# tohtsky/myFM

Hardware: AMD Instinct MI355X
Metric: Gibbs iterations/sec (rank=32) (higher is better)
Workload: dtype f64

## Files before the change

### myfm_amd/csrc/mfm_res.hpp

```cpp
#pragma once
#include <algorithm>
#include <cstdlib>
#include <cstring>
#include <atomic>
#include <string>
#include <thread>
#include <vector>

#include "mfm_common.hpp"
#include "mfm_mf_kernels.hpp"

namespace mfm {

#ifndef MFM_RES_CH
#define MFM_RES_CH 4
#endif
constexpr int RES_MAX_PEERS = 8;

struct ResArgs {
  double2 *eq;
  const double *e_in;
  double *e_slots;
  const int32_t *perm;
  const uint32_t *uidw;
  const uint32_t *headw;
  const int32_t *run_item;
  const int32_t *first_run;
  const int32_t *wg_run_ptr;
  const int32_t *wg_nruns;
  const int32_t *wg_user_ptr;
  const int2 *user_desc;
  const int32_t *wg_item_ptr;
  const int32_t *ent_ptr;
  const int2 *entries;
  const int32_t *scols;
  const int2 *item_desc;
  double *partials;
  double *dv;
  double *V;
  int64_t D;
  int f_begin, f_end;
  int linear;
  int n_sw;
  double *w;
  const double *zw;
  const double *lam_w, *mu_w;
  double e_shift;
  const double *z;
  const double *lam, *mu;
  const int32_t *group;
  int n_groups;
  double alpha;
  const double *scal;
  int n_items, umax;
  unsigned long long *bar;
  int n_wg;
  int *error;
  unsigned long long *prof;
  int xworld, xrank;
  unsigned long long xepoch0;
  double *xsum[RES_MAX_PEERS];
  unsigned long long *xflag[RES_MAX_PEERS];
  unsigned long long *xarrive;
  int xmodel;
  double *xw[RES_MAX_PEERS], *xV[RES_MAX_PEERS];
  int ngx;
  int no_store;
  int xch_break;
};

__device__ __forceinline__ void res_store2(double *p, double a, double b) {
  __hip_atomic_store(p, a, __ATOMIC_RELAXED, __HIP_MEMORY_SCOPE_AGENT);
  __hip_atomic_store(p + 1, b, __ATOMIC_RELAXED, __HIP_MEMORY_SCOPE_AGENT);
}

enum { RES_BAR_START = 0, RES_BAR_TOP = 16, RES_BAR_XCNT = 32, RES_BAR_GEN = 160, RES_BAR_CENSUS = 288, RES_BAR_WORDS = 416 };
struct ResBar {
  int xcc;
  unsigned long long n_x, nx;
};

__device__ __forceinline__ bool res_spin(const ResArgs &a, const unsigned long long *w, unsigned long long target, bool &dead) {
  unsigned spins = 0;
  while (__hip_atomic_load(w, __ATOMIC_RELAXED, __HIP_MEMORY_SCOPE_AGENT) < target) {
#ifndef MFM_RES_NO_SLEEP
    __builtin_amdgcn_s_sleep(1);
#endif
    if ((++spins & 1023u) == 0u) {
      if (spins > (1u << 22) || __hip_atomic_load(a.error, __ATOMIC_RELAXED, __HIP_MEMORY_SCOPE_AGENT) != 0) {
        __hip_atomic_store(a.error, 1, __ATOMIC_RELAXED, __HIP_MEMORY_SCOPE_AGENT);
        dead = true;
        return false;
      }
    }
  }
  return true;
}

__device__ __forceinline__ bool res_spin_sys(const ResArgs &a, const unsigned long long *w, unsigned long long target, bool &dead) {
  unsigned spins = 0;
  while (__hip_atomic_load(w, __ATOMIC_RELAXED, __HIP_MEMORY_SCOPE_SYSTEM) < target) {
    __builtin_amdgcn_s_sleep(2);
    if ((++spins & 1023u) == 0u) {
      const int seen = __hip_atomic_load(a.error, __ATOMIC_RELAXED, __HIP_MEMORY_SCOPE_AGENT);
      if (spins > (1u << 23) || seen != 0) {
        if (seen == 0) __hip_atomic_store(a.error, 2, __ATOMIC_RELAXED, __HIP_MEMORY_SCOPE_AGENT);
        dead = true;
        return false;
      }
    }
  }
  return true;
}

__device__ __forceinline__ void res_bar_init(const ResArgs &a, ResBar &rb, bool &dead) {
  unsigned x;
  asm volatile("s_getreg_b32 %0, hwreg(HW_REG_XCC_ID, 0, 4)" : "=s"(x));
  rb.xcc = (int)(x & 7u);
  __hip_atomic_fetch_add(a.bar + RES_BAR_CENSUS + 16 * rb.xcc, 1ull, __ATOMIC_RELAXED, __HIP_MEMORY_SCOPE_AGENT);
  asm volatile("s_waitcnt vmcnt(0)" ::: "memory");
  __hip_atomic_fetch_add(a.bar + RES_BAR_START, 1ull, __ATOMIC_RELAXED, __HIP_MEMORY_SCOPE_AGENT);
  rb.n_x = 1;
  rb.nx = 1;
  if (!res_spin(a, a.bar + RES_BAR_START, (unsigned long long)a.n_wg, dead)) return;
  rb.nx = 0;
  for (int i = 0; i < 8; i++) {
    const unsigned long long c = __hip_atomic_load(a.bar + RES_BAR_CENSUS + 16 * i, __ATOMIC_RELAXED, __HIP_MEMORY_SCOPE_AGENT);
    rb.nx += c > 0 ? 1 : 0;
    if (i == rb.xcc) rb.n_x = c;
  }
}

__device__ __forceinline__ void res_grid_barrier(const ResArgs &a, const ResBar &rb, unsigned long long k, int tid, bool &dead) {
  asm volatile("s_waitcnt vmcnt(0)" ::: "memory");
  __syncthreads();
  if (tid == 0 && !dead) {
    const unsigned long long old =
        __hip_atomic_fetch_add(a.bar + RES_BAR_XCNT + 16 * rb.xcc, 1ull, __ATOMIC_RELAXED, __HIP_MEMORY_SCOPE_AGENT);
    if (old + 1 == k * rb.n_x) {
      __builtin_amdgcn_fence(__ATOMIC_RELEASE, "agent");
      asm volatile("s_waitcnt vmcnt(0)" ::: "memory");
      __hip_atomic_fetch_add(a.bar + RES_BAR_TOP, 1ull, __ATOMIC_RELAXED, __HIP_MEMORY_SCOPE_AGENT);
      if (res_spin(a, a.bar + RES_BAR_TOP, k * rb.nx, dead))
        __hip_atomic_store(a.bar + RES_BAR_GEN + 16 * rb.xcc, k, __ATOMIC_RELAXED, __HIP_MEMORY_SCOPE_AGENT);
    } else {
      res_spin(a, a.bar + RES_BAR_GEN + 16 * rb.xcc, k, dead);
    }
    __builtin_amdgcn_fence(__ATOMIC_ACQUIRE, "agent");
  }
  __syncthreads();
}

typedef double res_d16_t __attribute__((ext_vector_type(16)));
typedef unsigned res_u4_t __attribute__((ext_vector_type(4)));

template <int NT, int NGV, int NGL, bool XCH = false, bool OVF = false>
__global__ __launch_bounds__(NT) void k_mf_resident(ResArgs a) {
  extern __shared__ __attribute__((aligned(16))) char res_smem[];
  constexpr int NW = NT / WAVE, NG = NGV + NGL, R = 16 * NG, RL = 16 * NGL;
  constexpr int B = 4;
  const int g = (int)blockIdx.x, tid = threadIdx.x, lane = tid & 63;
  const int wv = __builtin_amdgcn_readfirstlane(tid >> 6);
  const int U = a.umax;
  const double alpha_k = a.scal ? a.scal[0] : a.alpha, e_shift_k = a.scal ? a.scal[2] : a.e_shift;
  const int ngx = OVF ? a.ngx : 0, NGt = NG + ngx, Rt = 16 * NGt;
  double *elds = (double *)res_smem;
  double *acc1 = elds + (size_t)RL * NT;
  double *acc2 = acc1 + NW * U;
  d2_t *utab = (d2_t *)(acc2 + NW * U);
  d2_t *wcarry = utab + U;
  int *wflag = (int *)(wcarry + NW);
  const int32_t *perm_g = a.perm + (int64_t)g * Rt * NT;
  const d2_t *dv2 = (const d2_t *)a.dv;
  const int u0 = a.wg_user_ptr[g], nu = a.wg_user_ptr[g + 1] - u0;
  const int rb0 = a.wg_run_ptr[g];
  const int pad_item = a.n_items;
  bool dead = false;
  unsigned long long nbar = 0;
  ResBar rbar;
  rbar.xcc = 0;
  rbar.n_x = rbar.nx = 1;
#define RES_STAMP0(k) \
  if (a.prof && tid == 0) a.prof[(int64_t)g * a.n_sw * 64 + 56 + (k)] = __builtin_amdgcn_s_memrealtime()
  RES_STAMP0(0);
  if (tid == 0) res_bar_init(a, rbar, dead);
  RES_STAMP0(1);
  const int wv_hi = wv >> 2;
#define RES_PRIO(j)                  \
  if ((((j) & 1) ^ wv_hi) != 0)      \
    __builtin_amdgcn_s_setprio(1);   \
  else                               \
    __builtin_amdgcn_s_setprio(0)
  const int trash_run = a.wg_run_ptr[g] + a.wg_nruns[g];
#define RES_STAMP(k)                                                                                      \
  if (a.prof && tid == 0) a.prof[((int64_t)g * a.n_sw + (f - f_first)) * 64 + (k)] = __builtin_amdgcn_s_memrealtime()

  for (int i = tid; i < 2 * NW * U; i += NT) acc1[i] = 0.0;
  for (int i = tid; i < U; i += NT) utab[i] = d2_t{0.0, 0.0};

  res_u4_t uw[NG];
  unsigned ux[NG];
  unsigned hbv[NG], nbv[NG];
#pragma unroll
  for (int j = 0; j < NG; j++) {
#pragma unroll
    for (int w = 0; w < 4; w++) uw[j][w] = a.uidw[((int64_t)g * (5 * NGt) + 5 * j + w) * NT + tid];
    ux[j] = a.uidw[((int64_t)g * (5 * NGt) + 5 * j + 4) * NT + tid];
    hbv[j] = a.headw[((int64_t)g * NGt + j) * NT + tid];
    nbv[j] = hbv[j] | (j == 0 ? 1u : 0u);
  }
  const unsigned nbx0 = OVF && ngx > 0 ? a.headw[((int64_t)g * NGt + NG) * NT + tid] : 0u;
  double *eog = OVF ? a.e_slots + ((int64_t)g * Rt + 16 * NG) * NT + tid : nullptr;
  const uint32_t *uidw_x = a.uidw + ((int64_t)g * (5 * NGt) + 5 * NG) * NT + tid;
  const uint32_t *headw_x = a.headw + ((int64_t)g * NGt + NG) * NT + tid;
  const int run0 = a.first_run[g * NT + tid];
  const bool head0 = (hbv[0] & 1u) != 0u;
#define RES_NIB(j, q) ((((nbv[j]) | ((j) + 1 < NG ? nbv[(j) + 1 < NG ? (j) + 1 : (j)] << 16 : nbx0 << 16)) >> (4 * (q))) & 15u)
#define RES_UIDS(j, bb, uid)                                                     \
  {                                                                              \
    const unsigned lo_ = uw[j][bb];                                              \
    uid[0] = (int)(lo_ & 0x3ffu);                                                \
    uid[1] = (int)((lo_ >> 10) & 0x3ffu);                                        \
    uid[2] = (int)((lo_ >> 20) & 0x3ffu);                                        \
    uid[3] = (int)((lo_ >> 30) | (((ux[j] >> (8 * (bb))) & 0xffu) << 2));        \
  }

#define RES_UIDSX(bb, uid)                                                       \
  {                                                                              \
    const unsigned lo_ = uwx[bb];                                                \
    uid[0] = (int)(lo_ & 0x3ffu);                                                \
    uid[1] = (int)((lo_ >> 10) & 0x3ffu);                                        \
    uid[2] = (int)((lo_ >> 20) & 0x3ffu);                                        \
    uid[3] = (int)((lo_ >> 30) | (((uxx >> (8 * (bb))) & 0xffu) << 2));          \
  }

  res_d16_t ev[NGV > 0 ? NGV : 1];
#pragma unroll
  for (int j = 0; j < NG; j++) {
#pragma unroll 1
    for (int bb = 0; bb < 4; bb++) {
      int row[B];
#pragma unroll
      for (int k = 0; k < B; k++) row[k] = a.e_in ? 0 : perm_g[(16 * j + 4 * bb + k) * NT + tid];
#pragma unroll
      for (int k = 0; k < B; k++) {
        const double x = (a.e_in ? a.e_in[((int64_t)g * Rt + 16 * j + 4 * bb + k) * NT + tid] : a.eq[row[k] < 0 ? 0 : row[k]].x) + e_shift_k;
        if (j < NGV)
          ev[j < NGV ? j : 0][4 * bb + k] = x;
        else
          elds[(16 * (j - NGV) + 4 * bb + k) * NT + tid] = x;
      }
    }
  }
  if (OVF) {
    for (int jx = 0; jx < ngx; jx++) {
#pragma unroll 4
      for (int i = 0; i < 16; i++) {
        const int64_t sl = 16 * (NG + jx) + i;
        const int row = a.e_in ? 0 : perm_g[sl * NT + tid];
        const double x = (a.e_in ? a.e_in[((int64_t)g * Rt + sl) * NT + tid] : a.eq[row < 0 ? 0 : row].x) + e_shift_k;
        eog[(16 * jx + i) * NT] = x;
      }
    }
  }
  __syncthreads();

  RES_STAMP0(2);
  const int f_first = a.f_begin - a.linear;
  for (int f = f_first; f < a.f_end; f++) {
    const bool lin = f < a.f_begin;
    double *Vf = lin ? a.w : a.V + (int64_t)f * a.D;
    const double *zf = lin ? a.zw : a.z + (int64_t)(f - a.f_begin) * a.D;
    const double *lamf = lin ? a.lam_w : a.lam + (int64_t)f * a.n_groups;
    const double *muf = lin ? a.mu_w : a.mu + (int64_t)f * a.n_groups;
    int uj = 0;
    double uold = 0.0, uz = 0.0, ulam = 0.0, umu = 0.0;
    if (tid < nu) {
      const int2 d = a.user_desc[u0 + tid];
      uj = d.x;
      uold = Vf[uj];
      uz = zf[uj];
      ulam = lamf[d.y];
      umu = muf[d.y];
    }
    RES_STAMP(0);
    {
      int rc = run0 - 1;
      int itA[B];
      d2_t ddA[B];
      {
        int it0[B];
        const unsigned n0 = RES_NIB(0, 0), n1 = RES_NIB(0, 1);
#pragma unroll
        for (int k = 0; k < B; k++) {
          rc += (int)((n0 >> k) & 1u);
          it0[k] = a.run_item[(n0 >> k) & 1u ? rc : rb0];
        }
#pragma unroll
        for (int k = 0; k < B; k++) {
          rc += (int)((n1 >> k) & 1u);
          itA[k] = a.run_item[(n1 >> k) & 1u ? rc : rb0];
        }
#pragma unroll
        for (int k = 0; k < B; k++) ddA[k] = dv2[(n0 >> k) & 1u ? it0[k] : pad_item];
      }
      d2_t ddc = d2_t{0.0, 0.0};
      int itB[B];
      d2_t ddB[B];
#define RES_STEP_A(j, bb, iti, ito, ddi, ddo)                                                                              \
  {                                                                                                                        \
    const unsigned n4 = RES_NIB(j, bb), n4a = RES_NIB(j, (bb) + 1), n4b = RES_NIB(j, (bb) + 2);                            \
    _Pragma("unroll") for (int k = 0; k < B; k++) {                                                                        \
      rc += (int)((n4b >> k) & 1u);                                                                                        \
      ito[k] = a.run_item[(n4b >> k) & 1u ? rc : rb0];                                                                     \
    }                                                                                                                      \
    _Pragma("unroll") for (int k = 0; k < B; k++) ddo[k] = dv2[(n4a >> k) & 1u ? iti[k] : pad_item];                       \
    int uid[B];                                                                                                            \
    RES_UIDS(j, bb, uid);                                                                                                  \
    double up[B], ex[B];                                                                                                   \
    _Pragma("unroll") for (int k = 0; k < B; k++) {                                                                        \
      up[k] = utab[uid[k]][0];                                                                                             \
      ex[k] = j < NGV ? ev[j < NGV ? j : 0][4 * (bb) + k] : elds[(16 * (j - NGV) + 4 * (bb) + k) * NT + tid];              \
    }                                                                                                                      \
    _Pragma("unroll") for (int k = 0; k < B; k++) {                                                                        \
      const bool need = ((n4 >> k) & 1u) != 0u;                                                                            \
      ddc[0] = need ? ddi[k][0] : ddc[0];                                                                                  \
      ddc[1] = need ? ddi[k][1] : ddc[1];                                                                                  \
      const double er = ex[k] + up[k] * ddc[0];                                                                            \
      if (j < NGV)                                                                                                         \
        ev[j < NGV ? j : 0][4 * (bb) + k] = er;                                                                            \
      else                                                                                                                 \
        elds[(16 * (j - NGV) + 4 * (bb) + k) * NT + tid] = er;                                                             \
      const double c = ddc[1];                                                                                             \
      __hip_atomic_fetch_add(&acc1[wv * U + uid[k]], (-er) * c, __ATOMIC_RELAXED, __HIP_MEMORY_SCOPE_WORKGROUP);           \
      __hip_atomic_fetch_add(&acc2[wv * U + uid[k]], c * c, __ATOMIC_RELAXED, __HIP_MEMORY_SCOPE_WORKGROUP);               \
    }                                                                                                                      \
  }
#define RES_STEP_AX(bb, iti, ito, ddi, ddo)                                                                                 \
  {                                                                                                                        \
    const unsigned n4 = ((nbw >> (4 * (bb))) & 15u), n4a = ((nbw >> (4 * ((bb) + 1))) & 15u), n4b = ((nbw >> (4 * ((bb) + 2))) & 15u);                            \
    _Pragma("unroll") for (int k = 0; k < B; k++) {                                                                        \
      rc += (int)((n4b >> k) & 1u);                                                                                        \
      ito[k] = a.run_item[(n4b >> k) & 1u ? rc : rb0];                                                                     \
    }                                                                                                                      \
    _Pragma("unroll") for (int k = 0; k < B; k++) ddo[k] = dv2[(n4a >> k) & 1u ? iti[k] : pad_item];                       \
    int uid[B];                                                                                                            \
    RES_UIDSX(bb, uid);                                                                                                      \
    double up[B], ex[B];                                                                                                   \
    _Pragma("unroll") for (int k = 0; k < B; k++) {                                                                        \
      up[k] = utab[uid[k]][0];                                                                                             \
      ex[k] = eo[4 * (bb) + k];              \
    }                                                                                                                      \
    _Pragma("unroll") for (int k = 0; k < B; k++) {                                                                        \
      const bool need = ((n4 >> k) & 1u) != 0u;                                                                            \
      ddc[0] = need ? ddi[k][0] : ddc[0];                                                                                  \
      ddc[1] = need ? ddi[k][1] : ddc[1];                                                                                  \
      const double er = ex[k] + up[k] * ddc[0];                                                                            \
      eo[4 * (bb) + k] = er;                                                             \
      const double c = ddc[1];                                                                                             \
      __hip_atomic_fetch_add(&acc1[wv * U + uid[k]], (-er) * c, __ATOMIC_RELAXED, __HIP_MEMORY_SCOPE_WORKGROUP);           \
      __hip_atomic_fetch_add(&acc2[wv * U + uid[k]], c * c, __ATOMIC_RELAXED, __HIP_MEMORY_SCOPE_WORKGROUP);               \
    }                                                                                                                      \
  }
#pragma unroll
      for (int j = 0; j < NG; j++) {
        RES_PRIO(j);
#pragma unroll 1
        for (int bp = 0; bp < 2; bp++) {
          RES_STEP_A(j, 2 * bp, itA, itB, ddA, ddB);
          RES_STEP_A(j, 2 * bp + 1, itB, itA, ddB, ddA);
        }
      }
      if (OVF) {
        unsigned hb_c = nbx0;
        for (int jx = 0; jx < ngx; jx++) {
          res_u4_t uwx;
#pragma unroll
          for (int w = 0; w < 4; w++) uwx[w] = uidw_x[(5 * jx + w) * NT];
          const unsigned uxx = uidw_x[(5 * jx + 4) * NT];
          const unsigned hb_n = jx + 1 < ngx ? headw_x[(jx + 1) * NT] : 0u;
          const unsigned nbw = hb_c | (hb_n << 16);
          res_d16_t eo;
#pragma unroll
          for (int i = 0; i < 16; i++) eo[i] = eog[(16 * jx + i) * NT];
#pragma unroll 1
          for (int bp = 0; bp < 2; bp++) {
            RES_STEP_AX(2 * bp, itA, itB, ddA, ddB);
            RES_STEP_AX(2 * bp + 1, itB, itA, ddB, ddA);
          }
#pragma unroll
          for (int i = 0; i < 16; i++) eog[(16 * jx + i) * NT] = eo[i];
          hb_c = hb_n;
        }
      }
#undef RES_STEP_A
#undef RES_STEP_AX
    }
    __syncthreads();
    RES_STAMP(1);
    if (tid < nu) {
      double S1 = 0.0, S2 = 0.0;
#pragma unroll
      for (int w = 0; w < NW; w++) {
        S1 += acc1[w * U + tid];
        S2 += acc2[w * U + tid];
        acc1[w * U + tid] = 0.0;
        acc2[w * U + tid] = 0.0;
      }
      const double fresh = PMainV::draw(S1, S2, uold, alpha_k, ulam, umu, uz);
      Vf[uj] = fresh;
      if (XCH && a.xmodel) {
        for (int r = 0; r < a.xworld; r++)
          if (r != a.xrank)
            __hip_atomic_store((lin ? a.xw[r] : a.xV[r] + (int64_t)f * a.D) + uj, fresh, __ATOMIC_RELAXED, __HIP_MEMORY_SCOPE_SYSTEM);
      }
      utab[tid] = d2_t{lin ? 1.0 : fresh, fresh - uold};
    }
    __syncthreads();
    RES_STAMP(2);
    {
      bool have_head = false;
      double f1 = 0.0, f2 = 0.0, s1 = 0.0, s2 = 0.0;
      d2_t *part2 = (d2_t *)a.partials;
      {
        int rc = run0 - 1, rcC = run0 - 1;
        int itA[B];
        double ccA[B];
        {
          int it0[B];
          const unsigned n0 = RES_NIB(0, 0), n1 = RES_NIB(0, 1);
#pragma unroll
          for (int k = 0; k < B; k++) {
            rc += (int)((n0 >> k) & 1u);
            it0[k] = a.run_item[(n0 >> k) & 1u ? rc : rb0];
          }
#pragma unroll
          for (int k = 0; k < B; k++) {
            rc += (int)((n1 >> k) & 1u);
            itA[k] = a.run_item[(n1 >> k) & 1u ? rc : rb0];
          }
#pragma unroll
          for (int k = 0; k < B; k++) ccA[k] = a.dv[2 * (int64_t)((n0 >> k) & 1u ? it0[k] : pad_item) + 1];
        }
        double ccc = 0.0;
        int itB[B];
        double ccB[B];
#ifdef MFM_RES_UCST
#define RES_PARTIAL_STORE() part2[head && have_head ? rcC - 1 : trash_run] = d2_t{s1, s2}
#else
#define RES_PARTIAL_STORE() \
  if (head && have_head) part2[rcC - 1] = d2_t{s1, s2}
#endif
#define RES_STEP_B(j, bb, iti, ito, cci, cco)                                                                              \
  {                                                                                                                        \
    const unsigned n4 = RES_NIB(j, bb), n4a = RES_NIB(j, (bb) + 1), n4b = RES_NIB(j, (bb) + 2);                            \
    const unsigned h4 = (hbv[j] >> (4 * (bb))) & 15u;                                                                      \
    _Pragma("unroll") for (int k = 0; k < B; k++) {                                                                        \
      rc += (int)((n4b >> k) & 1u);                                                                                        \
      ito[k] = a.run_item[(n4b >> k) & 1u ? rc : rb0];                                                                     \
    }                                                                                                                      \
    _Pragma("unroll") for (int k = 0; k < B; k++) cco[k] = a.dv[2 * (int64_t)((n4a >> k) & 1u ? iti[k] : pad_item) + 1];   \
    int uid[B];                                                                                                            \
    RES_UIDS(j, bb, uid);                                                                                                  \
    d2_t ut[B];                                                                                                            \
    double ex[B];                                                                                                          \
    _Pragma("unroll") for (int k = 0; k < B; k++) {                                                                        \
      ut[k] = utab[uid[k]];                                                                                                \
      ex[k] = j < NGV ? ev[j < NGV ? j : 0][4 * (bb) + k] : elds[(16 * (j - NGV) + 4 * (bb) + k) * NT + tid];              \
    }                                                                                                                      \
    _Pragma("unroll") for (int k = 0; k < B; k++) {                                                                        \
      const bool need = ((n4 >> k) & 1u) != 0u;                                                                            \
      const bool head = ((h4 >> k) & 1u) != 0u;                                                                            \
      ccc = need ? cci[k] : ccc;                                                                                           \
      rcC += need ? 1 : 0;                                                                       \
                              \
      RES_PARTIAL_STORE();                                                                                                 \
      f1 = head && !have_head ? s1 : f1;                                                                                   \
      f2 = head && !have_head ? s2 : f2;                                                                                   \
      have_head = have_head || head;                                                                                       \
      const double er = ex[k] + ccc * ut[k][1];                                                                            \
      if (j < NGV)                                                                                                         \
        ev[j < NGV ? j : 0][4 * (bb) + k] = er;                                                                            \
      else                                                                                                                 \
        elds[(16 * (j - NGV) + 4 * (bb) + k) * NT + tid] = er;                                                             \
      s1 = (head ? 0.0 : s1) + (-er) * ut[k][0];                                                                           \
      s2 = (head ? 0.0 : s2) + ut[k][0] * ut[k][0];                                                                        \
    }                                                                                                                      \
  }
#define RES_STEP_BX(bb, iti, ito, cci, cco)                                                                                 \
  {                                                                                                                        \
    const unsigned n4 = ((nbw >> (4 * (bb))) & 15u), n4a = ((nbw >> (4 * ((bb) + 1))) & 15u), n4b = ((nbw >> (4 * ((bb) + 2))) & 15u);                            \
    const unsigned h4 = (hb_c >> (4 * (bb))) & 15u;                                                                       \
    _Pragma("unroll") for (int k = 0; k < B; k++) {                                                                        \
      rc += (int)((n4b >> k) & 1u);                                                                                        \
      ito[k] = a.run_item[(n4b >> k) & 1u ? rc : rb0];                                                                     \
    }                                                                                                                      \
    _Pragma("unroll") for (int k = 0; k < B; k++) cco[k] = a.dv[2 * (int64_t)((n4a >> k) & 1u ? iti[k] : pad_item) + 1];   \
    int uid[B];                                                                                                            \
    RES_UIDSX(bb, uid);                                                                                                      \
    d2_t ut[B];                                                                                                            \
    double ex[B];                                                                                                          \
    _Pragma("unroll") for (int k = 0; k < B; k++) {                                                                        \
      ut[k] = utab[uid[k]];                                                                                                \
      ex[k] = eo[4 * (bb) + k];              \
    }                                                                                                                      \
    _Pragma("unroll") for (int k = 0; k < B; k++) {                                                                        \
      const bool need = ((n4 >> k) & 1u) != 0u;                                                                            \
      const bool head = ((h4 >> k) & 1u) != 0u;                                                                            \
      ccc = need ? cci[k] : ccc;                                                                                           \
      rcC += need ? 1 : 0;                                                                       \
                              \
      RES_PARTIAL_STORE();                                                                                                 \
      f1 = head && !have_head ? s1 : f1;                                                                                   \
      f2 = head && !have_head ? s2 : f2;                                                                                   \
      have_head = have_head || head;                                                                                       \
      const double er = ex[k] + ccc * ut[k][1];                                                                            \
      eo[4 * (bb) + k] = er;                                                             \
      s1 = (head ? 0.0 : s1) + (-er) * ut[k][0];                                                                           \
      s2 = (head ? 0.0 : s2) + ut[k][0] * ut[k][0];                                                                        \
    }                                                                                                                      \
  }
#pragma unroll
        for (int j = 0; j < NG; j++) {
          RES_PRIO(j);
#pragma unroll 1
          for (int bp = 0; bp < 2; bp++) {
              RES_STEP_B(j, 2 * bp, itA, itB, ccA, ccB);
            if (a.prof && lane == 0 && (wv == 4 || wv == 7))
              a.prof[((int64_t)g * a.n_sw + (f - f_first)) * 64 + 16 + (wv == 4 ? 0 : 20) + 4 * j + 2 * bp] =
                  __builtin_amdgcn_s_memrealtime();
            RES_STEP_B(j, 2 * bp + 1, itB, itA, ccB, ccA);
            if (a.prof && lane == 0 && (wv == 4 || wv == 7))
              a.prof[((int64_t)g * a.n_sw + (f - f_first)) * 64 + 16 + (wv == 4 ? 0 : 20) + 4 * j + 2 * bp + 1] =
                  __builtin_amdgcn_s_memrealtime();
          }
        }
        if (OVF) {
          unsigned hb_c = nbx0;
          for (int jx = 0; jx < ngx; jx++) {
            res_u4_t uwx;
#pragma unroll
            for (int w = 0; w < 4; w++) uwx[w] = uidw_x[(5 * jx + w) * NT];
            const unsigned uxx = uidw_x[(5 * jx + 4) * NT];
            const unsigned hb_n = jx + 1 < ngx ? headw_x[(jx + 1) * NT] : 0u;
            const unsigned nbw = hb_c | (hb_n << 16);
            res_d16_t eo;
#pragma unroll
            for (int i = 0; i < 16; i++) eo[i] = eog[(16 * jx + i) * NT];
#pragma unroll 1
            for (int bp = 0; bp < 2; bp++) {
              RES_STEP_BX(2 * bp, itA, itB, ccA, ccB);
              RES_STEP_BX(2 * bp + 1, itB, itA, ccB, ccA);
            }
#pragma unroll
            for (int i = 0; i < 16; i++) eog[(16 * jx + i) * NT] = eo[i];
            hb_c = hb_n;
          }
        }
#undef RES_STEP_B
#undef RES_STEP_BX
#undef RES_PARTIAL_STORE
      }
      if (a.prof && lane == 0)
        a.prof[((int64_t)g * a.n_sw + (f - f_first)) * 64 + 8 + wv] = __builtin_amdgcn_s_memrealtime();
      double v1 = s1, v2 = s2;
      int fl = have_head ? 1 : 0;
      wave_segscan2(v1, v2, fl);
      if (lane == 63) {
        wcarry[wv] = d2_t{v1, v2};
        wflag[wv] = fl;
      }
      double x1 = dpp_f64<0x138, 0xf>(v1), x2 = dpp_f64<0x138, 0xf>(v2);
      int xf = dpp_i32<0x138, 0xf>(fl, 0);
      if (lane == 0) {
        x1 = 0.0;
        x2 = 0.0;
        xf = 0;
      }
      lds_barrier();
      if (have_head && tid > 0) {
        if (!xf) {
          double c1 = 0.0, c2 = 0.0;
          for (int w = 0; w < wv; w++) {
            const d2_t cw = wcarry[w];
            const bool fw = wflag[w] != 0;
            c1 = (fw ? 0.0 : c1) + cw[0];
            c2 = (fw ? 0.0 : c2) + cw[1];
          }
          x1 = c1 + x1;
          x2 = c2 + x2;
        }
        const int closing = head0 ? run0 - 1 : run0;
        part2[closing] = d2_t{x1 + f1, x2 + f2};
      }
    }
    RES_STAMP(3);
    constexpr int CH = MFM_RES_CH;
    const int c0 = a.ent_ptr[g] >> 6, c1 = a.ent_ptr[g + 1] >> 6;
    const int per = (c1 - c0 + NW - 1) / NW;
    const int wb = c0 + wv * per, we = wb + per < c1 ? wb + per : c1;
    const int i0 = a.wg_item_ptr[g], ni = a.wg_item_ptr[g + 1] - i0;
    const bool more = f + 1 < a.f_end;
    int ij = 0;
    double iold = 0.0, iz = 0.0, ivn = 0.0, ilam = 0.0, imu = 0.0;
    if (tid < ni) {
      const int2 d = a.item_desc[i0 + tid];
      ij = d.x;
      iold = Vf[ij];
      iz = zf[ij];
      ivn = more ? a.V[(int64_t)(f + 1) * a.D + ij] : 0.0;
      ilam = lamf[d.y];
      imu = muf[d.y];
    }
    int2 en[CH];
#pragma unroll
    for (int k = 0; k < CH; k++) en[k] = make_int2(0, 0);
    if (wb < we) {
#pragma unroll
      for (int k = 0; k < CH; k++) en[k] = a.entries[(int64_t)(wb + k < we ? wb + k : wb) * WAVE + lane];
    }
    res_grid_barrier(a, rbar, ++nbar, tid, dead);
    RES_STAMP(4);
    {
      const d2_t *part2 = (const d2_t *)a.partials;
      for (int cb = wb; cb < we; cb += CH) {
        d2_t sv[CH];
#pragma unroll
        for (int k = 0; k < CH; k++) sv[k] = part2[en[k].x];
        int il[CH];
#pragma unroll
        for (int k = 0; k < CH; k++) il[k] = en[k].y;
        if (cb + CH < we) {
#pragma unroll
          for (int k = 0; k < CH; k++) en[k] = a.entries[(int64_t)(cb + CH + k < we ? cb + CH + k : cb + CH) * WAVE + lane];
        }
#pragma unroll
        for (int k = 0; k < CH; k++) {
          if (cb + k >= we) break;
          __hip_atomic_fetch_add(&acc1[wv * U + il[k]], sv[k][0], __ATOMIC_RELAXED, __HIP_MEMORY_SCOPE_WORKGROUP);
          __hip_atomic_fetch_add(&acc2[wv * U + il[k]], sv[k][1], __ATOMIC_RELAXED, __HIP_MEMORY_SCOPE_WORKGROUP);
        }
      }
      __syncthreads();
      double S1 = 0.0, S2 = 0.0;
      if (tid < ni) {
#pragma unroll
        for (int w = 0; w < NW; w++) {
          S1 += acc1[w * U + tid];
          S2 += acc2[w * U + tid];
          acc1[w * U + tid] = 0.0;
          acc2[w * U + tid] = 0.0;
        }
      }
      if (XCH) {
        const unsigned long long E = a.xepoch0 + (unsigned long long)(f - f_first) + 1ull;
        const int64_t stride = 2 * ((int64_t)a.n_items + 1), par = (int64_t)(E & 1ull);
        if (tid < ni) {
          const int64_t off = ((int64_t)a.xrank * 2 + par) * stride + 2 * (int64_t)(i0 + tid);
          for (int r = 0; r < a.xworld; r++) {
            __hip_atomic_store(a.xsum[r] + off, S1, __ATOMIC_RELAXED, __HIP_MEMORY_SCOPE_SYSTEM);
            __hip_atomic_store(a.xsum[r] + off + 1, S2, __ATOMIC_RELAXED, __HIP_MEMORY_SCOPE_SYSTEM);
          }
        }
        asm volatile("s_waitcnt vmcnt(0)" ::: "memory");
        __syncthreads();
        if (tid == 0 && !dead) {
          const unsigned long long old = __hip_atomic_fetch_add(a.xarrive, 1ull, __ATOMIC_RELAXED, __HIP_MEMORY_SCOPE_AGENT);
          if (old + 1 == (unsigned long long)a.n_wg * E) {
            for (int r = 0; r < a.xworld && !a.xch_break; r++)
              __hip_atomic_store(a.xflag[r] + 16 * a.xrank, E, __ATOMIC_RELEASE, __HIP_MEMORY_SCOPE_SYSTEM);
          }
          for (int r = 0; r < a.xworld && !dead; r++) res_spin_sys(a, a.xflag[a.xrank] + 16 * r, E, dead);
        }
        __syncthreads();
        if (tid < ni) {
          S1 = S2 = 0.0;
          for (int r = 0; r < a.xworld; r++) {
            const int64_t off = ((int64_t)r * 2 + par) * stride + 2 * (int64_t)(i0 + tid);
            S1 += __hip_atomic_load(a.xsum[a.xrank] + off, __ATOMIC_RELAXED, __HIP_MEMORY_SCOPE_SYSTEM);
            S2 += __hip_atomic_load(a.xsum[a.xrank] + off + 1, __ATOMIC_RELAXED, __HIP_MEMORY_SCOPE_SYSTEM);
          }
        }
      }
      if (tid < ni) {
        const double fresh = PMainV::draw(S1, S2, iold, alpha_k, ilam, imu, iz);
        Vf[ij] = fresh;
        res_store2(a.dv + 2 * (int64_t)(i0 + tid), fresh - iold, ivn);
      }
    }
    RES_STAMP(5);
    res_grid_barrier(a, rbar, ++nbar, tid, dead);
    RES_STAMP(6);
  }
#undef RES_STAMP
  RES_STAMP0(3);
  if (!a.no_store) {
    int run_last = run0;
#pragma unroll
    for (int j = 0; j < NG; j++) {
#pragma unroll 1
      for (int bb = 0; bb < 4; bb++) {
        const unsigned h4 = (hbv[j] >> (4 * bb)) & 15u;
        int row[B], it[B];
#pragma unroll
        for (int k = 0; k < B; k++) {
          if (16 * j + 4 * bb + k > 0) run_last += (int)((h4 >> k) & 1u);
          it[k] = a.run_item[run_last];
          row[k] = perm_g[(16 * j + 4 * bb + k) * NT + tid];
        }
        int uid[B];
        RES_UIDS(j, bb, uid);
#pragma unroll
        for (int k = 0; k < B; k++) {
          const double dl = a.dv[2 * (int64_t)it[k]];
          const double ex = j < NGV ? ev[j < NGV ? j : 0][4 * bb + k] : elds[(16 * (j - NGV) + 4 * bb + k) * NT + tid];
          const double ef = ex + utab[uid[k]][0] * dl;
          if (a.e_slots)
            a.e_slots[((int64_t)g * Rt + 16 * j + 4 * bb + k) * NT + tid] = ef;
          else if (row[k] >= 0)
            a.eq[row[k]].x = ef;
        }
      }
    }
    if (OVF) {
      for (int jx = 0; jx < ngx; jx++) {
        res_u4_t uwx;
#pragma unroll
        for (int w = 0; w < 4; w++) uwx[w] = uidw_x[(5 * jx + w) * NT];
        const unsigned uxx = uidw_x[(5 * jx + 4) * NT];
        const unsigned hbx = headw_x[jx * NT];
#pragma unroll 1
        for (int bb = 0; bb < 4; bb++) {
          const unsigned h4 = (hbx >> (4 * bb)) & 15u;
          int it[B], uid[B];
#pragma unroll
          for (int k = 0; k < B; k++) {
            run_last += (int)((h4 >> k) & 1u);
            it[k] = a.run_item[run_last];
          }
          RES_UIDSX(bb, uid);
#pragma unroll
          for (int k = 0; k < B; k++) {
            const double dl = a.dv[2 * (int64_t)it[k]];
            double *ep = eog + (16 * jx + 4 * bb + k) * NT;
            *ep = *ep + utab[uid[k]][0] * dl;
          }
        }
      }
    }
  }
#undef RES_PRIO
#undef RES_NIB
#undef RES_UIDS
#undef RES_UIDSX
  asm volatile("s_waitcnt vmcnt(0)" ::: "memory");
  RES_STAMP0(4);
#undef RES_STAMP0
}

__global__ void k_res_init_dv(const double *__restrict__ theta, const int32_t *__restrict__ scols, int n_items,
                              double *__restrict__ dv, unsigned long long *__restrict__ bar) {
  const int i = blockIdx.x * blockDim.x + threadIdx.x;
  if (blockIdx.x == 0)
    for (int k = threadIdx.x; k < RES_BAR_WORDS; k += blockDim.x) bar[k] = 0ull;
  if (i < n_items) {
    dv[2 * i] = 0.0;
    dv[2 * i + 1] = theta ? theta[scols[i]] : 1.0;
  } else if (i == n_items) {
    dv[2 * i] = 0.0;
    dv[2 * i + 1] = 0.0;
  }
}

__global__ void k_res_unpermute(const double *__restrict__ e_slots, const int32_t *__restrict__ perm, int64_t n_slots,
                                double2 *__restrict__ eq) {
  const int64_t i = (int64_t)blockIdx.x * blockDim.x + threadIdx.x;
  if (i >= n_slots) return;
  const int32_t row = perm[i];
  if (row >= 0) eq[row].x = e_slots[i];
}

struct ResScoreArgs {
  const uint32_t *uidw, *headw;
  const int32_t *first_run, *run_feat, *wg_user_ptr, *wg_fill;
  const int2 *user_desc;
  int umax, KS;
  const double *Vt, *w;
  double w0;
  const double *w0p;
  const double *y_slots;
  double *e_slots;
  double2 *sums;
  unsigned long long *prof;
};

template <int NT, int NG, int KPT>
__global__ __launch_bounds__(NT) void k_res_score(ResScoreArgs a) {
  extern __shared__ __attribute__((aligned(16))) char res_smem[];
  constexpr int R = 16 * NG, NW = NT / WAVE;
  constexpr int US = 2 * KPT + 2;
  const int g = blockIdx.x, tid = threadIdx.x, lane = tid & 63, wv = tid >> 6;
  const int KP = a.KS >> 1;
  const double w0_k = a.w0p ? *a.w0p : a.w0;
  double *uV = (double *)res_smem;
  double *uW = uV + (size_t)a.umax * US;
  double2 *wsum = (double2 *)(uW + ((a.umax + 1) & ~1));
  if (a.prof && tid == 0) a.prof[4 * g] = __builtin_amdgcn_s_memrealtime();
  int *ucol = (int *)(wsum + NW);
  const int u0 = a.wg_user_ptr[g], nu = a.wg_user_ptr[g + 1] - u0;
  for (int ul = tid; ul < a.umax; ul += NT) {
    const int ju = ul < nu ? a.user_desc[u0 + ul].x : -1;
    ucol[ul] = ju;
    uW[ul] = ju >= 0 ? a.w[ju] : 0.0;
  }
  __syncthreads();
#pragma unroll 4
  for (int i = tid; i < a.umax * KPT; i += NT) {
    const int ul = i / KPT, pr = i - ul * KPT;
    const int ju = ucol[ul];
    double2 v = make_double2(0.0, 0.0);
    if (ju >= 0 && pr < KP) v = ((const double2 *)(a.Vt + (int64_t)ju * a.KS))[pr];
    ((double2 *)(uV + (size_t)ul * US))[pr] = v;
  }
  res_u4_t uw[NG];
  unsigned ux[NG], hbv[NG];
#pragma unroll
  for (int j = 0; j < NG; j++) {
#pragma unroll
    for (int w = 0; w < 4; w++) uw[j][w] = a.uidw[((int64_t)g * (5 * NG) + 5 * j + w) * NT + tid];
    ux[j] = a.uidw[((int64_t)g * (5 * NG) + 5 * j + 4) * NT + tid];
    hbv[j] = a.headw[((int64_t)g * NG + j) * NT + tid];
  }
  int run = a.first_run[g * NT + tid];
  const int64_t fill = a.wg_fill[g];
  __syncthreads();
  if (a.prof && tid == 0) a.prof[4 * g + 1] = __builtin_amdgcn_s_memrealtime();
  double2 vi[KPT];
  double wi = 0.0, s1 = 0.0, s2 = 0.0;
#pragma unroll
  for (int p = 0; p < KPT; p++) vi[p] = make_double2(0.0, 0.0);
  int jc[4], jn[4];
  double yn[4];
#pragma unroll
  for (int k = 0; k < 4; k++) yn[k] = a.y_slots[((int64_t)g * R + k) * NT + tid];
  {
    const unsigned h0 = hbv[0] & 15u;
    int r = run;
#pragma unroll
    for (int k = 0; k < 4; k++) {
      if (k > 0) r += (int)((h0 >> k) & 1u);
      jc[k] = a.run_feat[r];
    }
    run = r;
  }
#pragma unroll
  for (int j = 0; j < NG; j++) {
    const unsigned hb2 = hbv[j] | (j + 1 < NG ? hbv[j + 1 < NG ? j + 1 : j] << 16 : 0u);
#pragma unroll 1
    for (int bb = 0; bb < 4; bb++) {
      {
        const unsigned hn = (hb2 >> (4 * (bb + 1))) & 15u;
        int r = run;
#pragma unroll
        for (int k = 0; k < 4; k++) {
          r += (int)((hn >> k) & 1u);
          jn[k] = a.run_feat[r];
        }
        run = r;
      }
      const unsigned lo_ = uw[j][bb];
      int uid[4];
      uid[0] = (int)(lo_ & 0x3ffu);
      uid[1] = (int)((lo_ >> 10) & 0x3ffu);
      uid[2] = (int)((lo_ >> 20) & 0x3ffu);
      uid[3] = (int)((lo_ >> 30) | (((ux[j] >> (8 * bb)) & 0xffu) << 2));
      const unsigned h4 = (hbv[j] >> (4 * bb)) & 15u;
      double yv[4], eb[4];
#pragma unroll
      for (int k = 0; k < 4; k++) yv[k] = yn[k];
      {
        const int nb = 16 * j + 4 * bb + 4 < R ? 16 * j + 4 * bb + 4 : 0;
#pragma unroll
        for (int k = 0; k < 4; k++) yn[k] = a.y_slots[((int64_t)g * R + nb + k) * NT + tid];
      }
#pragma unroll
      for (int k = 0; k < 4; k++) {
        const int slot = 16 * j + 4 * bb + k;
        const bool head = slot == 0 || ((h4 >> k) & 1u);
        if (head) {
          const int ji = jc[k];
          wi = 0.0;
          if (ji >= 0) {
            const double2 *src = (const double2 *)(a.Vt + (int64_t)ji * a.KS);
#pragma unroll
            for (int p = 0; p < KPT; p++) vi[p] = p < KP ? src[p] : make_double2(0.0, 0.0);
            wi = a.w[ji];
          } else {
#pragma unroll
            for (int p = 0; p < KPT; p++) vi[p] = make_double2(0.0, 0.0);
          }
        }
        const double2 *vu = (const double2 *)(uV + (size_t)uid[k] * US);
        double d0 = 0.0, d1 = 0.0;
#pragma unroll
        for (int p = 0; p < KPT; p += 2) {
          const double2 x0 = vu[p], x1 = vu[p + 1];
          d0 += x0.x * vi[p].x + x0.y * vi[p].y;
          d1 += x1.x * vi[p + 1].x + x1.y * vi[p + 1].y;
        }
        const double pred = w0_k + (uW[uid[k]] + wi) + (d0 + d1);
        const bool real = (int64_t)tid * R + slot < fill;
        const double e = real ? pred - yv[k] : 0.0;
        eb[k] = e;
        s1 += e;
        s2 += e * e;
      }
#pragma unroll
      for (int k = 0; k < 4; k++) a.e_slots[((int64_t)g * R + 16 * j + 4 * bb + k) * NT + tid] = eb[k];
#pragma unroll
      for (int k = 0; k < 4; k++) jc[k] = jn[k];
    }
  }
  if (a.prof && lane == 0) a.prof[4 * g + 2] = __builtin_amdgcn_s_memrealtime();
  wave_allreduce_sum2(s1, s2);
  if (lane == 0) wsum[wv] = make_double2(s1, s2);
  __syncthreads();
  if (a.prof && tid == 0) a.prof[4 * g + 3] = __builtin_amdgcn_s_memrealtime();
  if (tid == 0) {
    double t1 = 0.0, t2 = 0.0;
    for (int w = 0; w < NW; w++) {
      t1 += wsum[w].x;
      t2 += wsum[w].y;
    }
    a.sums[g] = make_double2(t1, t2);
  }
}

__global__ void k_res_permute_y(const double *__restrict__ y, const int32_t *__restrict__ perm, int64_t n_slots,
                                double *__restrict__ y_slots) {
  const int64_t i = (int64_t)blockIdx.x * blockDim.x + threadIdx.x;
  if (i >= n_slots) return;
  const int32_t row = perm[i];
  y_slots[i] = row >= 0 ? y[row] : 0.0;
}

template <class F>
static inline void res_parallel_for(int n, F f) {
  const int hw = (int)std::thread::hardware_concurrency();
  const int T = std::max(1, std::min({n, 16, hw > 0 ? hw : 1}));
  if (T == 1) {
    for (int i = 0; i < n; i++) f(i);
    return;
  }
  std::atomic<int> next(0);
  auto work = [&]() {
    for (;;) {
      const int i = next.fetch_add(1);
      if (i >= n) return;
      f(i);
    }
  };
  std::vector<std::thread> pool;
  for (int t = 1; t < T; t++) pool.emplace_back(work);
  work();
  for (auto &t : pool) t.join();
}

struct ResPlan {
  bool ready = false;
  int G = 0, NT = 512, RV = 0, RL = 0, umax = 0, item_bits = 0, n_items = 0;
  int RX = 0;
  int R() const { return RV + RL + RX; }
  bool allow_overflow = true;
  int64_t n_rows = 0, n_runs = 0;
  size_t lds_bytes = 0;
  DevBuf<int32_t> perm, first_run, wg_run_ptr, wg_nruns, wg_user_ptr, wg_item_ptr, ent_ptr, scols;
  DevBuf<int2> entries;
  DevBuf<uint32_t> uidw, headw;
  DevBuf<int32_t> run_item;
  DevBuf<int2> user_desc, item_desc;
  DevBuf<double> partials, dv, e_slots;
  DevBuf<unsigned long long> bar;
  DevBuf<int32_t> run_feat, wg_fill;
  DevBuf<double> y_slots;
  DevBuf<double2> sums;
  int maxu_rows = 0;
  int xworld = 1, xrank = 0;
  bool peers_set = false;
  DevBuf<double> xsum;
  DevBuf<unsigned long long> xflag, xarrive;
  double *peer_sum[RES_MAX_PEERS] = {nullptr, nullptr, nullptr, nullptr, nullptr, nullptr, nullptr, nullptr};
  unsigned long long *peer_flag[RES_MAX_PEERS] = {nullptr, nullptr, nullptr, nullptr, nullptr, nullptr, nullptr, nullptr};
  unsigned long long xepoch = 0;
  bool peers_model = false;
  double *peer_w[RES_MAX_PEERS] = {nullptr, nullptr, nullptr, nullptr, nullptr, nullptr, nullptr, nullptr};
  double *peer_V[RES_MAX_PEERS] = {nullptr, nullptr, nullptr, nullptr, nullptr, nullptr, nullptr, nullptr};
  std::vector<void *> peer_mapped;
  size_t xsum_bytes(int world) const { return (size_t)world * 2 * 2 * ((size_t)n_items + 1) * sizeof(double); }
  void alloc_exchange(int world, int rank, hipStream_t s) {
    xworld = world;
    xrank = rank;
    peers_set = false;
    peers_model = false;
    xepoch = 0;
    auto alloc_shared = [&](auto &buf, size_t count) {
      buf.release();
      void *p = nullptr;
      const size_t bytes = count * sizeof(*buf.p);
      if (hipExtMallocWithFlags(&p, bytes, hipDeviceMallocUncached) != hipSuccess) {
        (void)hipGetLastError();
        throw Error(MFM_ERR_DEVICE, "no uncached device memory for the ranks' exchange buffers (hipExtMallocWithFlags(hipDeviceMallocUncached))");
      }
      buf.p = (decltype(buf.p))p;
      buf.n = count;
      buf.owned = true;
      MFM_HIP_CHECK(hipMemsetAsync(p, 0, bytes, s));
    };
    alloc_shared(xsum, xsum_bytes(world) / sizeof(double));
    alloc_shared(xflag, (size_t)16 * RES_MAX_PEERS);
    xarrive.alloc_zero(16, s);
  }
  std::string why;
  std::vector<int32_t> h_nruns;
  std::vector<std::string> h_diag;

  static int bits_for(int64_t n) {
    int b = 1;
    while (((int64_t)1 << b) < n) b++;
    return b;
  }
  struct Variant {
    int rv, rl;
  };
  static const Variant *variants(int &n) {
    static const Variant v[] = {{16, 0}, {32, 0}, {64, 16}};
    n = 3;
    return v;
  }

  bool choose_layout(int64_t N, const std::vector<int64_t> &ustart, int64_t max_user, int n_cu, std::vector<int64_t> &ucut) {
    const int64_t n_users = (int64_t)ustart.size() - 1;
    int nv = 0;
    const Variant *vs = variants(nv);
    bool found = false;
    for (int vi = 0; vi < nv && !found; vi++) {
      const int64_t cap = (int64_t)NT * (vs[vi].rv + vs[vi].rl) - 1;
      if (max_user > cap) continue;
      const int64_t slack = std::min<int64_t>(cap / 8, max_user);
      int64_t Gw = (N + (cap - slack) - 1) / (cap - slack);
      if (Gw > n_cu && N <= (int64_t)n_cu * cap) Gw = n_cu;
      if (Gw > n_cu) continue;
      if (env_flag("MFM_RES_WGS")) Gw = std::min<int64_t>(n_cu, std::max<int64_t>(Gw, env_i64("MFM_RES_WGS", 0)));
      Gw = std::min<int64_t>(Gw, n_users);
      ucut.assign(1, 0);
      bool ok = true;
      for (int64_t g = 1; g <= Gw && ok; g++) {
        const int64_t lo_u = ucut.back();
        int64_t hi_u;
        if (g == Gw) {
          hi_u = n_users;
        } else {
          const int64_t want = (N * g) / Gw;
          hi_u = std::upper_bound(ustart.begin(), ustart.end(), want) - ustart.begin() - 1;
          if (hi_u + 1 <= n_users && ustart[hi_u + 1] - want < want - ustart[hi_u]) hi_u++;
          hi_u = std::max(hi_u, lo_u + 1);
          hi_u = std::min<int64_t>(hi_u, n_users - (Gw - g));
          while (hi_u > lo_u + 1 && ustart[hi_u] - ustart[lo_u] > cap) hi_u--;
        }
        if (hi_u <= lo_u || ustart[hi_u] - ustart[lo_u] > cap) ok = false;
        ucut.push_back(hi_u);
      }
      if (!ok) continue;
      G = (int)Gw;
      RV = vs[vi].rv;
      RL = vs[vi].rl;
      found = true;
    }
    RX = 0;
    if (!found && allow_overflow) {
      const Variant big = vs[nv - 1];
      for (int rx = 16; rx <= 80 && !found; rx += 16) {
        const int64_t cap = (int64_t)NT * (big.rv + big.rl + rx) - 1;
        if (max_user > cap || N > (int64_t)n_cu * cap) continue;
        int64_t Gw = std::min<int64_t>(n_cu, n_users);
        ucut.assign(1, 0);
        bool ok = true;
        for (int64_t g = 1; g <= Gw && ok; g++) {
          const int64_t lo_u = ucut.back();
          int64_t hi_u;
          if (g == Gw) {
            hi_u = n_users;
          } else {
            const int64_t want = (N * g) / Gw;
            hi_u = std::upper_bound(ustart.begin(), ustart.end(), want) - ustart.begin() - 1;
            if (hi_u + 1 <= n_users && ustart[hi_u + 1] - want < want - ustart[hi_u]) hi_u++;
            hi_u = std::max(hi_u, lo_u + 1);
            hi_u = std::min<int64_t>(hi_u, n_users - (Gw - g));
            while (hi_u > lo_u + 1 && ustart[hi_u] - ustart[lo_u] > cap) hi_u--;
          }
          if (hi_u <= lo_u || ustart[hi_u] - ustart[lo_u] > cap) ok = false;
          ucut.push_back(hi_u);
        }
        if (!ok) continue;
        G = (int)Gw;
        RV = big.rv;
        RL = big.rl;
        RX = rx;
        found = true;
      }
    }
    if (!found) return fail("no variant fits (rows per CU, or a first-level column longer than a workgroup's capacity)");
    return true;
  }
  bool choose_item_slices(const std::vector<int32_t> &slot_ptr, int64_t counter, std::vector<int32_t> &iptr) {
    iptr.assign((size_t)G + 1, 0);
    bool ok = false;
    for (double scale = 1.0; scale < 3.0 && !ok; scale *= 1.1) {
      const double target = scale * ((double)counter + 16.0 * n_items) / G;
      double acc = 0.0;
      int gq = 0, cnt = 0;
      for (int c = 0; c < n_items; c++) {
        acc += (double)(slot_ptr[c + 1] - slot_ptr[c]) + 16.0;
        cnt++;
        if ((acc >= target || cnt == NT) && gq + 1 < G) {
          iptr[++gq] = c + 1;
          acc = 0.0;
          cnt = 0;
        }
      }
      ok = cnt <= NT;
      for (gq++; gq <= G; gq++) iptr[gq] = n_items;
    }
    if (!ok) return fail("more second-level columns than the workgroups can draw");
    return true;
  }
  static std::vector<int32_t> run_bases(const std::vector<int32_t> &nruns) {
    const int G = (int)nruns.size();
    std::vector<int32_t> run_base((size_t)G + 1, 0);
    for (int g = 0; g < G; g++) run_base[g + 1] = run_base[g] + nruns[g] + 1;
    return run_base;
  }

  bool build(const HostCsr &csc, const std::vector<int32_t> &level, const std::vector<int32_t> *group_of, int n_cu,
             const std::vector<char> *draw_empty = nullptr) {
    ready = false;
    const int64_t N = csc.cols, D0 = csc.rows;
    n_rows = N;
    if (N < 1 || n_cu < 1 || (int64_t)level.size() != D0) return fail("shape");
    std::vector<int32_t> users, items, empties;
    for (int64_t j = 0; j < D0; j++) {
      if (level[j] == 0) {
        if (csc.ptr[j + 1] > csc.ptr[j])
          users.push_back((int32_t)j);
        else if (!draw_empty || (*draw_empty)[(size_t)j])
          empties.push_back((int32_t)j);
      } else if (level[j] == 1) {
        items.push_back((int32_t)j);
      } else {
        return fail("more than two levels");
      }
    }
    n_items = (int)items.size();
    if (users.empty() || items.empty()) return fail("empty level");
    std::sort(users.begin(), users.end(), [&](int32_t x, int32_t y) { return csc.idx[csc.ptr[x]] < csc.idx[csc.ptr[y]]; });
    std::vector<int64_t> ustart(users.size() + 1);
    int64_t next_row = 0, max_user = 0;
    for (size_t u = 0; u < users.size(); u++) {
      const int32_t j = users[u];
      const int64_t b = csc.ptr[j], len = csc.ptr[j + 1] - b;
      if (csc.idx[b] != next_row || csc.idx[b + len - 1] != next_row + len - 1) return fail("first level not contiguous");
      ustart[u] = next_row;
      next_row += len;
      max_user = std::max(max_user, len);
    }
    ustart[users.size()] = next_row;
    if (next_row != N) return fail("first level does not cover the rows");
    std::vector<int32_t> item_of_row((size_t)N, -1);
    {
      int64_t cnt = 0;
      for (int c = 0; c < n_items; c++) cnt += csc.ptr[items[c] + 1] - csc.ptr[items[c]];
      if (cnt != N) return fail("second level does not cover the rows");
      const int chunks = std::max(1, std::min(n_items, 64));
      res_parallel_for(chunks, [&](int k) {
        for (int c = (int)((int64_t)n_items * k / chunks); c < (int)((int64_t)n_items * (k + 1) / chunks); c++)
          for (int64_t p = csc.ptr[items[c]]; p < csc.ptr[items[c] + 1]; p++) item_of_row[csc.idx[p]] = c;
      });
      std::atomic<bool> bad(false);
      res_parallel_for(chunks, [&](int k) {
        for (int64_t r = N * k / chunks; r < N * (k + 1) / chunks; r++)
          if (item_of_row[r] < 0) bad = true;
      });
      if (bad) return fail("second level touches a row twice");
    }
    std::vector<int64_t> ucut;
    if (!choose_layout(N, ustart, max_user, n_cu, ucut)) return false;
    const int R = RV + RL + RX;
    const int64_t cap_slots = (int64_t)NT * R;
    std::vector<std::vector<int32_t>> wg_users((size_t)G);
    for (int g = 0; g < G; g++)
      for (int64_t u = ucut[g]; u < ucut[g + 1]; u++) wg_users[g].push_back(users[u]);
    for (size_t k = 0; k < empties.size(); k++) wg_users[k % G].push_back(empties[k]);
    int maxu = 0;
    for (int g = 0; g < G; g++) maxu = std::max(maxu, (int)wg_users[g].size());
    if (maxu > NT) return fail("more first-level columns in a workgroup than threads");
    item_bits = bits_for((int64_t)n_items + 1);
    const int UW = 5 * (R / 16), HW = R / 16;
    std::vector<uint16_t> h_uid((size_t)G * cap_slots, 0xffffu);
    std::vector<uint32_t> h_headw((size_t)G * HW * NT, 0);
    std::vector<int32_t> h_perm((size_t)G * cap_slots, -1), h_first((size_t)G * NT, 0);
    std::vector<std::vector<int32_t>> wg_run_item((size_t)G);
    std::vector<int64_t> fill((size_t)G, 0);
    std::vector<int32_t> nruns((size_t)G, 0);
    res_parallel_for(G, [&](int g) {
      const int64_t row0 = ustart[ucut[g]], row1 = ustart[ucut[g + 1]];
      const int64_t n = row1 - row0;
      std::vector<int32_t> cnt((size_t)n_items + 1, 0), uloc((size_t)n);
      for (int64_t u = ucut[g]; u < ucut[g + 1]; u++)
        for (int64_t r = ustart[u]; r < ustart[u + 1]; r++) uloc[(size_t)(r - row0)] = (int32_t)(u - ucut[g]);
      for (int64_t r = row0; r < row1; r++) cnt[(size_t)item_of_row[r] + 1]++;
      std::vector<int32_t> &runs = wg_run_item[g];
      for (int c = 0; c < n_items; c++) {
        if (cnt[c + 1]) {
          const int64_t sidx = cnt[c];
          const int th = (int)(sidx / R), rh = (int)(sidx % R);
          h_headw[((size_t)g * HW + rh / 16) * NT + th] |= 1u << (rh % 16);
          runs.push_back(c);
        }
        cnt[c + 1] += cnt[c];
      }
      {
        size_t ri = 0;
        std::vector<int32_t> run_start(runs.size());
        for (size_t k = 0; k < runs.size(); k++) run_start[k] = cnt[runs[k]];
        for (int t = 0; t < NT; t++) {
          const int64_t s0 = (int64_t)t * R;
          if (s0 >= n) break;
          while (ri + 1 < runs.size() && run_start[ri + 1] <= s0) ri++;
          h_first[(size_t)g * NT + t] = (int32_t)ri;
        }
      }
      for (int64_t r = row0; r < row1; r++) {
        const int64_t sidx = cnt[(size_t)item_of_row[r]]++;
        const int t = (int)(sidx / R), rr = (int)(sidx % R);
        h_perm[(size_t)g * cap_slots + (size_t)rr * NT + t] = (int32_t)r;
        h_uid[(size_t)g * cap_slots + (size_t)sidx] = (uint16_t)uloc[(size_t)(r - row0)];
      }
      fill[g] = n;
      nruns[g] = (int32_t)runs.size();
    });
    std::vector<int32_t> h_slot_ptr((size_t)n_items + 1, 0);
    int64_t counter = 0;
    for (int g = 0; g < G; g++) {
      counter += nruns[g];
      for (int32_t c : wg_run_item[g]) h_slot_ptr[(size_t)c + 1]++;
    }
    for (int c = 0; c < n_items; c++) h_slot_ptr[(size_t)c + 1] += h_slot_ptr[c];
    h_slot_ptr[n_items] = (int32_t)counter;
    n_runs = counter;
    if (counter >= ((int64_t)1 << 31) - 2) return fail("too many runs");
    std::vector<int32_t> run_base = run_bases(nruns);
    const int32_t zero_run = run_base[G];
    std::vector<int32_t> h_run_item((size_t)zero_run + 1, n_items);
    for (int g = 0; g < G; g++) {
      std::copy(wg_run_item[g].begin(), wg_run_item[g].end(), h_run_item.begin() + run_base[g]);
      if (fill[g] < cap_slots) {
        const int th = (int)(fill[g] / R), rh = (int)(fill[g] % R);
        h_headw[((size_t)g * HW + rh / 16) * NT + th] |= 1u << (rh % 16);
      }
      h_headw[((size_t)g * HW) * NT] |= 1u;
      for (int t = 0; t < NT; t++) {
        const int64_t s0 = (int64_t)t * R;
        int32_t &fr = h_first[(size_t)g * NT + t];
        fr = (s0 >= fill[g] ? nruns[g] : fr) + run_base[g];
      }
    }
    std::vector<int32_t> h_uptr((size_t)G + 1, 0);
    std::vector<int2> h_udesc;
    for (int g = 0; g < G; g++) {
      for (int32_t j : wg_users[g]) h_udesc.push_back(make_int2(j, group_of && (size_t)j < group_of->size() ? (*group_of)[j] : 0));
      h_uptr[g + 1] = (int32_t)h_udesc.size();
    }
    std::vector<int32_t> h_iptr;
    if (!choose_item_slices(h_slot_ptr, counter, h_iptr)) return false;
    int imax = 0;
    for (int g = 0; g < G; g++) imax = std::max(imax, h_iptr[g + 1] - h_iptr[g]);
    umax = std::max(maxu, imax) + 1;
    if (umax > 1024) return fail("internal: user field");
    std::vector<uint32_t> h_uidw((size_t)G * UW * NT, 0);
    res_parallel_for(G, [&](int g) {
      for (int64_t sl = 0; sl < cap_slots; sl++) {
        const uint16_t u16 = h_uid[(size_t)g * cap_slots + (size_t)sl];
        const uint32_t u = u16 == 0xffffu ? (uint32_t)(umax - 1) : u16;
        const int t = (int)(sl / R), r = (int)(sl % R);
        const int w0 = 5 * (r / 16), bb = (r % 16) / 4, k = r % 4;
        if (k < 3) {
          h_uidw[((size_t)g * UW + w0 + bb) * NT + t] |= u << (10 * k);
        } else {
          h_uidw[((size_t)g * UW + w0 + bb) * NT + t] |= (u & 3u) << 30;
          h_uidw[((size_t)g * UW + w0 + 4) * NT + t] |= (u >> 2) << (8 * bb);
        }
      }
    });
    h_uid = std::vector<uint16_t>();
    std::vector<int32_t> slice_of((size_t)n_items);
    for (int g = 0; g < G; g++)
      for (int c = h_iptr[g]; c < h_iptr[g + 1]; c++) slice_of[c] = g;
    std::vector<int32_t> h_eptr((size_t)G + 1, 0);
    {
      std::vector<int64_t> cnt((size_t)G, 0);
      for (int g = 0; g < G; g++)
        for (int32_t c : wg_run_item[g]) cnt[slice_of[c]]++;
      for (int g = 0; g < G; g++) {
        const int64_t e = h_eptr[g] + ((cnt[g] + WAVE - 1) / WAVE) * WAVE;
        if (e >= ((int64_t)1 << 31)) return fail("too many entries");
        h_eptr[g + 1] = (int32_t)e;
      }
    }
    std::vector<int2> h_entries((size_t)h_eptr[G], make_int2(zero_run, 0));
    {
      std::vector<int64_t> pos((size_t)G);
      for (int g = 0; g < G; g++) pos[g] = h_eptr[g];
      for (int g = 0; g < G; g++)
        for (size_t l = 0; l < wg_run_item[g].size(); l++) {
          const int32_t c = wg_run_item[g][l];
          const int sgl = slice_of[c];
          h_entries[(size_t)pos[sgl]++] = make_int2(run_base[g] + (int32_t)l, c - h_iptr[sgl]);
        }
    }
    if (h_entries.size() >= ((size_t)1 << 31)) return fail("too many entries");
    lds_bytes = (size_t)RL * NT * 8 + (size_t)2 * (NT / WAVE) * umax * 8 + (size_t)umax * 16 + (size_t)(NT / WAVE) * 16 + (NT / WAVE) * 4 + 64;
    if (lds_bytes > 160 * 1024 - 512) return fail("LDS");
    uidw.upload(h_uidw);
    headw.upload(h_headw);
    run_item.upload(h_run_item);
    perm.upload(h_perm);
    first_run.upload(h_first);
    wg_user_ptr.upload(h_uptr);
    user_desc.upload(h_udesc.data(), h_udesc.size());
    wg_item_ptr.upload(h_iptr);
    ent_ptr.upload(h_eptr);
    entries.upload(h_entries.data(), h_entries.size());
    wg_run_ptr.upload(run_base);
    wg_nruns.upload(nruns);
    e_slots.alloc((size_t)G * cap_slots);
    {
      std::vector<int32_t> h_run_feat(h_run_item.size() + 8, -1);
      for (size_t r = 0; r < h_run_item.size(); r++) h_run_feat[r] = h_run_item[r] < n_items ? items[(size_t)h_run_item[r]] : -1;
      run_feat.upload(h_run_feat);
      std::vector<int32_t> h_fill((size_t)G);
      for (int g = 0; g < G; g++) h_fill[g] = (int32_t)fill[g];
      wg_fill.upload(h_fill);
      sums.alloc((size_t)G);
      y_slots = DevBuf<double>();
    }
    h_nruns = nruns;
    if (env_flag("MFM_RES_PROF")) {
      h_diag.assign((size_t)G, "");
      for (int g = 0; g < G; g++) {
        int64_t maxlen = 0;
        for (int64_t u = ucut[g]; u < ucut[g + 1]; u++) maxlen = std::max(maxlen, ustart[u + 1] - ustart[u]);
        int64_t sinstr = 0, maxst = 0, nthr_head = 0;
        for (int w = 0; w < NT / WAVE; w++) {
          std::vector<char> hh(WAVE, 0);
          std::vector<int> st(WAVE, 0);
          for (int r = 0; r < R; r++) {
            bool any = false;
            for (int l = 0; l < WAVE; l++) {
              const int t = w * WAVE + l;
              const bool head = (h_headw[((size_t)g * HW + r / 16) * NT + t] >> (r % 16)) & 1u;
              if (head && hh[l]) {
                any = true;
                st[l]++;
              }
              hh[l] = hh[l] || head;
            }
            sinstr += any;
          }
          for (int l = 0; l < WAVE; l++) {
            maxst = std::max<int64_t>(maxst, st[l]);
            nthr_head += hh[l];
          }
        }
        char buf[160];
        std::snprintf(buf, sizeof buf, "users %d maxlen %lld rows %lld store-instr %lld max-stores/thread %lld threads-with-head %lld",
                      (int)(ucut[g + 1] - ucut[g]), (long long)maxlen, (long long)fill[g], (long long)sinstr, (long long)maxst,
                      (long long)nthr_head);
        h_diag[g] = buf;
      }
    }
    scols.upload(items);
    {
      std::vector<int2> h_idesc(items.size());
      for (size_t i = 0; i < items.size(); i++) {
        const int32_t j = items[i];
        h_idesc[i] = make_int2(j, group_of && (size_t)j < group_of->size() ? (*group_of)[j] : 0);
      }
      item_desc.upload(h_idesc.data(), h_idesc.size());
    }
    partials.alloc((size_t)2 * ((size_t)zero_run + 1));
    MFM_HIP_CHECK(hipMemset(partials.p, 0, (size_t)16 * ((size_t)zero_run + 1)));
    dv.alloc((size_t)2 * (n_items + 1));
    bar.alloc(RES_BAR_WORDS);
    ready = true;
    why.clear();
    return true;
  }
  bool fail(const char *w) {
    why = w;
    ready = false;
    return false;
  }
};

static inline hipError_t res_occupancy(const ResPlan &rp, int *per_cu) {
  *per_cu = 0;
  const void *fn = nullptr;
  if (rp.RV == 16 && rp.RL == 0)
    fn = (const void *)k_mf_resident<512, 1, 0>;
  else if (rp.RV == 32 && rp.RL == 0)
    fn = (const void *)k_mf_resident<512, 2, 0>;
  else if (rp.RV == 64 && rp.RL == 16)
    fn = rp.RX ? (const void *)k_mf_resident<512, 4, 1, false, true> : (const void *)k_mf_resident<512, 4, 1>;
  else
    return hipErrorInvalidValue;
  hipError_t e = hipFuncSetAttribute(fn, hipFuncAttributeMaxDynamicSharedMemorySize, 160 * 1024);
  if (e != hipSuccess) return e;
  return hipOccupancyMaxActiveBlocksPerMultiprocessor(per_cu, fn, 512, rp.lds_bytes);
}

static inline void run_sweep_resident(hipStream_t s, Timing &tm, ResPlan &rp, int kernel_class, double2 *eq, double *V, int64_t D,
                                      int f_begin, int f_end, const double *zbase, const double *lam, const double *mu,
                                      const int32_t *group, int n_groups, double alpha, int *error,
                                      double *w = nullptr, const double *zw = nullptr, const double *lam_w = nullptr,
                                      const double *mu_w = nullptr, double e_shift = 0.0, bool load_slots = false,
                                      bool no_store = false, const double *scal = nullptr) {
  ResArgs a;
  std::memset(&a, 0, sizeof(a));
  a.scal = scal;
  a.eq = eq;
  a.e_slots = rp.e_slots.p;
  a.ngx = rp.RX / 16;
  a.no_store = no_store ? 1 : 0;
  a.e_in = load_slots ? rp.e_slots.p : nullptr;
  a.linear = w ? 1 : 0;
  a.n_sw = f_end - f_begin + a.linear;
  a.w = w;
  a.zw = zw;
  a.lam_w = lam_w;
  a.mu_w = mu_w;
  a.e_shift = e_shift;
  a.perm = rp.perm.p;
  a.uidw = rp.uidw.p;
  a.headw = rp.headw.p;
  a.run_item = rp.run_item.p;
  a.first_run = rp.first_run.p;
  a.wg_user_ptr = rp.wg_user_ptr.p;
  a.user_desc = rp.user_desc.p;
  a.wg_item_ptr = rp.wg_item_ptr.p;
  a.ent_ptr = rp.ent_ptr.p;
  a.entries = rp.entries.p;
  a.wg_run_ptr = rp.wg_run_ptr.p;
  a.wg_nruns = rp.wg_nruns.p;
  a.scols = rp.scols.p;
  a.item_desc = rp.item_desc.p;
  a.partials = rp.partials.p;
  a.dv = rp.dv.p;
  a.V = V;
  a.D = D;
  a.f_begin = f_begin;
  a.f_end = f_end;
  a.z = zbase;
  a.lam = lam;
  a.mu = mu;
  a.group = group;
  a.n_groups = n_groups;
  a.alpha = alpha;
  a.n_items = rp.n_items;
  a.umax = rp.umax;
  a.bar = rp.bar.p;
  a.n_wg = rp.G;
  a.error = error;
  const bool xch = rp.xworld > 1;
  a.xch_break = xch && rp.xrank == 1 && env_flag("MFM_RES_XCH_BREAK");
  a.xworld = rp.xworld;
  a.xrank = rp.xrank;
  a.xepoch0 = rp.xepoch;
  a.xarrive = rp.xarrive.p;
  a.xmodel = xch && rp.peers_model ? 1 : 0;
  for (int r = 0; r < RES_MAX_PEERS; r++) {
    a.xsum[r] = rp.peer_sum[r];
    a.xflag[r] = rp.peer_flag[r];
    a.xw[r] = rp.peer_w[r];
    a.xV[r] = rp.peer_V[r];
  }
  if (xch && !rp.peers_set) throw Error(MFM_ERR_RUNTIME, "row-sharded persistent sweep: the peers' exchange buffers are not set (mfm_peer_set)");
  static int prof_launch = 0;
  const bool prof = env_flag("MFM_RES_PROF") && ++prof_launch == env_int("MFM_RES_PROF", 0);
  DevBuf<unsigned long long> prof_buf;
  if (prof) {
    prof_buf.alloc((size_t)rp.G * a.n_sw * 64);
    MFM_HIP_CHECK(hipMemsetAsync(prof_buf.p, 0, (size_t)rp.G * a.n_sw * 512, s));
    a.prof = prof_buf.p;
  }
  const int K = a.n_sw;
  double bytes = (8.0 + (load_slots ? 0.0 : 4.0) + 1.4 + (no_store ? 0.0 : 8.0)) * rp.n_rows + K * 48.0 * rp.n_runs;
  if (rp.RX) bytes += (double)K * (16.0 + 1.75) * (double)rp.G * rp.NT * rp.RX;
  hipLaunchKernelGGL(k_res_init_dv, dim3((rp.n_items + 256) / 256), dim3(256), 0, s,
                     w ? (const double *)nullptr : V + (int64_t)f_begin * D, rp.scols.p, rp.n_items,
                     rp.dv.p, rp.bar.p);
  TimedLaunch t(tm, s, kernel_class, bytes);
#define MFM_RES_LAUNCH(RV_, RL_)                                                                                              \
  do {                                                                                                                        \
    static DeviceOnce raised;                                                                                                 \
    if (raised.need()) {                                                                                                      \
      MFM_HIP_CHECK(hipFuncSetAttribute((const void *)k_mf_resident<512, RV_ / 16, RL_ / 16>,                                  \
                                        hipFuncAttributeMaxDynamicSharedMemorySize, 160 * 1024));                             \
      raised.mark();                                                                                                          \
    }                                                                                                                         \
    if (xch) {                                                                                                                \
      static DeviceOnce raised_x;                                                                                             \
      if (raised_x.need()) {                                                                                                  \
        MFM_HIP_CHECK(hipFuncSetAttribute((const void *)k_mf_resident<512, RV_ / 16, RL_ / 16, true>,                          \
                                          hipFuncAttributeMaxDynamicSharedMemorySize, 160 * 1024));                           \
        raised_x.mark();                                                                                                      \
      }                                                                                                                       \
      hipLaunchKernelGGL((k_mf_resident<512, RV_ / 16, RL_ / 16, true>), dim3(rp.G), dim3(512), rp.lds_bytes, s, a);            \
    } else {                                                                                                                  \
      hipLaunchKernelGGL((k_mf_resident<512, RV_ / 16, RL_ / 16>), dim3(rp.G), dim3(512), rp.lds_bytes, s, a);                  \
    }                                                                                                                         \
  } while (0)
  if (rp.RV == 16 && rp.RL == 0)
    MFM_RES_LAUNCH(16, 0);
  else if (rp.RV == 32 && rp.RL == 0)
    MFM_RES_LAUNCH(32, 0);
  else if (rp.RV == 64 && rp.RL == 16 && rp.RX > 0) {
    if (xch) throw Error(MFM_ERR_RUNTIME, "internal: no row-sharded resident kernel with overflow slots");
    static DeviceOnce raised_o;
    if (raised_o.need()) {
      MFM_HIP_CHECK(hipFuncSetAttribute((const void *)k_mf_resident<512, 4, 1, false, true>, hipFuncAttributeMaxDynamicSharedMemorySize, 160 * 1024));
      raised_o.mark();
    }
    hipLaunchKernelGGL((k_mf_resident<512, 4, 1, false, true>), dim3(rp.G), dim3(512), rp.lds_bytes, s, a);
  } else if (rp.RV == 64 && rp.RL == 16)
    MFM_RES_LAUNCH(64, 16);
  else
    throw Error(MFM_ERR_RUNTIME, "internal: no resident kernel variant for this plan");
#undef MFM_RES_LAUNCH
  MFM_HIP_CHECK(hipGetLastError());
  if (xch) rp.xepoch += (unsigned long long)a.n_sw;
  if (prof) {
    MFM_HIP_CHECK(hipStreamSynchronize(s));
    const int K2 = a.n_sw;
    std::vector<unsigned long long> h((size_t)rp.G * K2 * 64);
    MFM_HIP_CHECK(hipMemcpy(h.data(), prof_buf.p, h.size() * 8, hipMemcpyDeviceToHost));
    const char *names[6] = {"sweep A", "user draw", "sweep B", "barrier 1 (wait)", "item draw", "barrier 2 (wait)"};
    std::fprintf(stderr, "[resident profile] G=%d factors=%d; us per factor: mean | mean of max over workgroups | mean of min\n", rp.G, K2);
    for (int ph = 0; ph < 6; ph++) {
      double sm = 0, smax = 0, smin = 0;
      for (int f = 0; f < K2; f++) {
        double mx = 0, mn = 1e30;
        for (int g = 0; g < rp.G; g++) {
          const unsigned long long *t = &h[((size_t)g * K2 + f) * 64];
          const double d = (double)(t[ph + 1] - t[ph]) * 0.01;
          sm += d;
          mx = std::max(mx, d);
          mn = std::min(mn, d);
        }
        smax += mx;
        smin += mn;
      }
      std::fprintf(stderr, "  %-18s %8.2f | %8.2f | %8.2f\n", names[ph], sm / ((double)rp.G * K2), smax / K2, smin / K2);
    }
    {
      std::vector<std::pair<double, int>> tb;
      for (int g = 0; g < rp.G; g++) {
        double d = 0;
        for (int f = 0; f < K2; f++) d += (double)(h[((size_t)g * K2 + f) * 64 + 3] - h[((size_t)g * K2 + f) * 64 + 2]) * 0.01;
        tb.push_back({d / K2, g});
      }
      std::sort(tb.begin(), tb.end());
      std::fprintf(stderr, "  sweep B by workgroup: fastest");
      for (int k = 0; k < 4; k++) std::fprintf(stderr, " wg %d %.1f (%d runs)", tb[k].second, tb[k].first, rp.h_nruns[tb[k].second]);
      std::fprintf(stderr, "; median wg %d %.1f (%d runs); slowest", tb[rp.G / 2].second, tb[rp.G / 2].first, rp.h_nruns[tb[rp.G / 2].second]);
      for (int k = rp.G - 4; k < rp.G; k++) std::fprintf(stderr, " wg %d %.1f (%d runs)", tb[k].second, tb[k].first, rp.h_nruns[tb[k].second]);
      std::fprintf(stderr, "\n");
      if (!rp.h_diag.empty())
        for (int k : {0, 1, rp.G / 2, rp.G - 3, rp.G - 2, rp.G - 1})
        {
          const int g = tb[k].second;
          std::fprintf(stderr, "    wg %d %.1f us: %s; waves:", g, tb[k].first, rp.h_diag[g].c_str());
          for (int w = 0; w < 8; w++) {
            double d = 0;
            for (int f = 0; f < K2; f++) d += (double)(h[((size_t)g * K2 + f) * 64 + 8 + w] - h[((size_t)g * K2 + f) * 64 + 2]) * 0.01;
            std::fprintf(stderr, " %.1f", d / K2);
          }
          std::fprintf(stderr, "\n      batches of waves 4 and 7 (factor 3 alone):");
          for (int w : {0, 20}) {
            std::fprintf(stderr, " |");
            for (int b = 0; b < (rp.RV + rp.RL) / 4; b++)
              std::fprintf(stderr, " %.1f", (double)(h[((size_t)g * K2 + 3) * 64 + 16 + w + b] - h[((size_t)g * K2 + 3) * 64 + 2]) * 0.01);
          }
          std::fprintf(stderr, "\n");
        }
    }
    if (const char *dump = env_str("MFM_RES_PROF_DUMP")) {
      if (FILE *fp = std::fopen(dump, "w")) {
        for (int g = 0; g < rp.G; g++) {
          std::fprintf(fp, "%d", g);
          for (int ph = 0; ph < 6; ph++) {
            double d = 0;
            for (int f = 0; f < K2; f++) d += (double)(h[((size_t)g * K2 + f) * 64 + ph + 1] - h[((size_t)g * K2 + f) * 64 + ph]) * 0.01;
            std::fprintf(fp, " %.2f", d / K2);
          }
          std::fprintf(fp, " | %s\n", rp.h_diag.empty() ? "" : rp.h_diag[g].c_str());
        }
        std::fclose(fp);
      }
    }
    {
      const char *nm[4] = {"census barrier", "residual load", "factor loop", "residual store"};
      for (int ph = 0; ph < 4; ph++) {
        double sm = 0, mx = 0;
        for (int g = 0; g < rp.G; g++) {
          const double d = (double)(h[(size_t)g * K2 * 64 + 56 + ph + 1] - h[(size_t)g * K2 * 64 + 56 + ph]) * 0.01;
          sm += d;
          mx = std::max(mx, d);
        }
        std::fprintf(stderr, "  %-18s %8.2f mean | %8.2f max (us, whole launch)\n", nm[ph], sm / rp.G, mx);
      }
      unsigned long long t0 = ~0ull, t1 = 0;
      for (int g = 0; g < rp.G; g++) {
        t0 = std::min(t0, h[(size_t)g * K2 * 64 + 56]);
        t1 = std::max(t1, h[(size_t)g * K2 * 64 + 60]);
      }
      std::fprintf(stderr, "  first workgroup in to last workgroup out: %.1f us\n", (double)(t1 - t0) * 0.01);
    }
    double tot = 0;
    for (int g = 0; g < rp.G; g++) tot += (double)(h[((size_t)g * K2 + K2 - 1) * 64 + 6] - h[(size_t)g * K2 * 64]) * 0.01;
    std::fprintf(stderr, "  factors, start to end: %.1f us (%.2f per factor)\n", tot / rp.G, tot / rp.G / K2);
  }
}

static inline bool res_score_supported(const ResPlan &rp, int K) {
  const int KS = (K + 1) & ~1;
  if (!rp.ready || K < 1 || KS > 32) return false;
  const size_t lds = ((size_t)rp.umax * (2 * 16 + 2) + ((rp.umax + 1) & ~1)) * 8 + 8 * 16 + (size_t)rp.umax * 4 + 64;
  return lds <= 160 * 1024 - 512;
}

static inline void run_res_score(hipStream_t s, Timing &tm, ResPlan &rp, int kernel_class, const double *Vt, const double *w,
                                 double w0, int K, const double *y, int64_t nnz, const double *w0p = nullptr) {
  const int KS = (K + 1) & ~1;
  const int64_t n_slots = (int64_t)rp.G * rp.R() * 512;
  if (!rp.y_slots.p) {
    rp.y_slots.alloc((size_t)n_slots);
    hipLaunchKernelGGL(k_res_permute_y, dim3((unsigned)((n_slots + 255) / 256)), dim3(256), 0, s, y, rp.perm.p, n_slots,
                       rp.y_slots.p);
  }
  ResScoreArgs a;
  a.uidw = rp.uidw.p;
  a.headw = rp.headw.p;
  a.first_run = rp.first_run.p;
  a.run_feat = rp.run_feat.p;
  a.wg_user_ptr = rp.wg_user_ptr.p;
  a.wg_fill = rp.wg_fill.p;
  a.user_desc = rp.user_desc.p;
  a.umax = rp.umax;
  a.KS = KS;
  a.Vt = Vt;
  a.w = w;
  a.w0 = w0;
  a.w0p = w0p;
  a.y_slots = rp.y_slots.p;
  a.e_slots = rp.e_slots.p;
  a.sums = rp.sums.p;
  static int prof_calls = 0;
  const bool prof = env_flag("MFM_RES_SCORE_PROF") && ++prof_calls == env_int("MFM_RES_SCORE_PROF", 0);
  DevBuf<unsigned long long> prof_buf;
  a.prof = nullptr;
  if (prof) {
    prof_buf.alloc((size_t)rp.G * 4);
    a.prof = prof_buf.p;
  }
  const size_t lds = ((size_t)rp.umax * (2 * 16 + 2) + ((rp.umax + 1) & ~1)) * 8 + 8 * 16 + (size_t)rp.umax * 4 + 64;
  TimedLaunch t(tm, s, kernel_class, 17.4 * rp.n_rows + 8.0 * KS * (double)rp.n_runs);
  (void)nnz;
#define MFM_RES_SCORE(NG_)                                                                                              \
  do {                                                                                                                  \
    static DeviceOnce raised;                                                                                           \
    if (raised.need()) {                                                                                                \
      MFM_HIP_CHECK(hipFuncSetAttribute((const void *)k_res_score<512, NG_, 16>, hipFuncAttributeMaxDynamicSharedMemorySize, \
                                        160 * 1024));                                                                   \
      raised.mark();                                                                                                    \
    }                                                                                                                   \
    hipLaunchKernelGGL((k_res_score<512, NG_, 16>), dim3(rp.G), dim3(512), lds, s, a);                                   \
  } while (0)
  const int NG = rp.R() / 16;
  if (NG == 1)
    MFM_RES_SCORE(1);
  else if (NG == 2)
    MFM_RES_SCORE(2);
  else if (NG == 5)
    MFM_RES_SCORE(5);
  else if (NG == 6)
    MFM_RES_SCORE(6);
  else if (NG == 7)
    MFM_RES_SCORE(7);
  else if (NG == 8)
    MFM_RES_SCORE(8);
  else if (NG == 9)
    MFM_RES_SCORE(9);
  else if (NG == 10)
    MFM_RES_SCORE(10);
  else
    throw Error(MFM_ERR_RUNTIME, "internal: no slot-order scorer for this plan");
#undef MFM_RES_SCORE
  MFM_HIP_CHECK(hipGetLastError());
  if (prof) {
    MFM_HIP_CHECK(hipStreamSynchronize(s));
    std::vector<unsigned long long> h((size_t)rp.G * 4);
    MFM_HIP_CHECK(hipMemcpy(h.data(), prof_buf.p, h.size() * 8, hipMemcpyDeviceToHost));
    unsigned long long t0 = ~0ull, t1 = 0;
    double st = 0, lp = 0, en = 0;
    for (int g = 0; g < rp.G; g++) {
      t0 = std::min(t0, h[4 * g]);
      t1 = std::max(t1, h[4 * g + 3]);
      st += (double)(h[4 * g + 1] - h[4 * g]) * 0.01;
      lp += (double)(h[4 * g + 2] - h[4 * g + 1]) * 0.01;
      en += (double)(h[4 * g + 3] - h[4 * g + 2]) * 0.01;
    }
    std::fprintf(stderr, "[k_res_score] first start to last end %.1f us; per workgroup (mean): users staged %.1f, slots %.1f, reduction %.1f us\n",
                 (double)(t1 - t0) * 0.01, st / rp.G, lp / rp.G, en / rp.G);
  }
}

}
```

### myfm_amd/csrc/mfm_res_plan.hpp

```cpp
#pragma once
#include <chrono>

#include <hipcub/hipcub.hpp>

#include "mfm_res.hpp"

namespace mfm {

namespace rp {

constexpr int TB = 256;

__global__ void k_rows(const int32_t *__restrict__ colidx, int64_t N, int32_t *__restrict__ bflag, int32_t *__restrict__ ucnt,
                       int32_t *__restrict__ icnt, int32_t *__restrict__ red) {
  const int64_t r = (int64_t)blockIdx.x * blockDim.x + threadIdx.x;
  int32_t mu = -1, mi = 0x7fffffff;
  if (r < N) {
    const int2 c = ((const int2 *)colidx)[r];
    const bool b = r == 0 || c.x != colidx[2 * (r - 1)];
    bflag[r] = b ? 1 : 0;
    if (b) atomicAdd(&ucnt[c.x], 1);
    atomicAdd(&icnt[c.y], 1);
    mu = c.x;
    mi = c.y;
  }
  for (int off = 32; off > 0; off >>= 1) {
    mu = max(mu, __shfl_xor(mu, off));
    mi = min(mi, __shfl_xor(mi, off));
  }
  if ((threadIdx.x & 63) == 0) {
    atomicMax(&red[0], mu);
    atomicMin(&red[1], mi);
  }
}

__global__ void k_cols(const int32_t *__restrict__ ucnt, const int32_t *__restrict__ icnt, int64_t D0, int32_t *__restrict__ iflag,
                       int32_t *__restrict__ eflag, int32_t *__restrict__ red) {
  const int64_t j = (int64_t)blockIdx.x * blockDim.x + threadIdx.x;
  if (j >= D0) return;
  const int32_t u = ucnt[j], i = icnt[j];
  if (u > 1 || (u > 0 && i > 0)) atomicAdd(&red[2], 1);
  iflag[j] = i > 0;
  eflag[j] = u == 0 && i == 0;
}

__global__ void k_cols_given(const int32_t *__restrict__ ucnt, const int32_t *__restrict__ icnt, const int32_t *__restrict__ level,
                             const int32_t *__restrict__ draw_empty, int64_t D0, int32_t *__restrict__ iflag, int32_t *__restrict__ eflag,
                             int32_t *__restrict__ red) {
  const int64_t j = (int64_t)blockIdx.x * blockDim.x + threadIdx.x;
  if (j >= D0) return;
  const int32_t u = ucnt[j], i = icnt[j], l = level[j];
  if (u > 1 || (u > 0 && l != 0) || (i > 0 && l != 1) || l < 0 || l > 1) atomicAdd(&red[2], 1);
  iflag[j] = l == 1;
  eflag[j] = l == 0 && u == 0 && draw_empty[j] != 0;
}

__global__ void k_col_lists(const int32_t *__restrict__ iflag, const int32_t *__restrict__ eflag, const int32_t *__restrict__ iord,
                            const int32_t *__restrict__ eord, int64_t D0, int32_t *__restrict__ scols, int32_t *__restrict__ empties) {
  const int64_t j = (int64_t)blockIdx.x * blockDim.x + threadIdx.x;
  if (j >= D0) return;
  if (iflag[j]) scols[iord[j]] = (int32_t)j;
  if (eflag[j]) empties[eord[j]] = (int32_t)j;
}

__global__ void k_users(const int32_t *__restrict__ colidx, const int32_t *__restrict__ bflag, const int32_t *__restrict__ uord1,
                        int64_t N, int32_t *__restrict__ ustart, int32_t *__restrict__ users) {
  const int64_t r = (int64_t)blockIdx.x * blockDim.x + threadIdx.x;
  if (r >= N) return;
  if (bflag[r]) {
    ustart[uord1[r] - 1] = (int32_t)r;
    users[uord1[r] - 1] = colidx[2 * r];
  }
  if (r == N - 1) ustart[uord1[r]] = (int32_t)N;
}

__device__ __forceinline__ int upper_group(const int32_t *cut, int G, int32_t x) {
  int lo = 0, hi = G;
  while (hi - lo > 1) {
    const int mid = (lo + hi) >> 1;
    if (cut[mid] <= x)
      lo = mid;
    else
      hi = mid;
  }
  return lo;
}

__global__ void k_keys(const int32_t *__restrict__ colidx, const int32_t *__restrict__ iord, const int32_t *__restrict__ rowcut, int G,
                       int item_bits, int64_t N, uint32_t *__restrict__ key, int32_t *__restrict__ val) {
  __shared__ int32_t cut[1026];
  for (int i = threadIdx.x; i <= G; i += blockDim.x) cut[i] = rowcut[i];
  __syncthreads();
  const int64_t r = (int64_t)blockIdx.x * blockDim.x + threadIdx.x;
  if (r >= N) return;
  const int g = upper_group(cut, G, (int32_t)r);
  key[r] = ((uint32_t)g << item_bits) | (uint32_t)iord[colidx[2 * r + 1]];
  val[r] = (int32_t)r;
}

__global__ void k_slots(const uint32_t *__restrict__ key, const int32_t *__restrict__ val, const int32_t *__restrict__ uord1,
                        const int32_t *__restrict__ rowcut, const int32_t *__restrict__ ucut, int item_bits, int R, int NT, int64_t N,
                        int32_t *__restrict__ perm, uint16_t *__restrict__ uid, int32_t *__restrict__ headf) {
  const int64_t p = (int64_t)blockIdx.x * blockDim.x + threadIdx.x;
  if (p >= N) return;
  const uint32_t k = key[p];
  const int g = (int)(k >> item_bits);
  const int32_t row = val[p];
  const int64_t cap = (int64_t)R * NT;
  const int32_t sidx = (int32_t)(p - rowcut[g]);
  const int t = sidx / R, rr = sidx % R;
  perm[(int64_t)g * cap + (int64_t)rr * NT + t] = row;
  uid[(int64_t)g * cap + sidx] = (uint16_t)(uord1[row] - 1 - ucut[g]);
  headf[p] = (sidx == 0 || k != key[p - 1]) ? 1 : 0;
}

__global__ void k_wg_runs(const int32_t *__restrict__ hs, const int32_t *__restrict__ rowcut, int G, int32_t *__restrict__ hrun0) {
  const int g = blockIdx.x * blockDim.x + threadIdx.x;
  if (g > G) return;
  hrun0[g] = rowcut[g] > 0 ? hs[rowcut[g] - 1] : 0;
}

__global__ void k_fill32(int32_t *p, int64_t n, int32_t v) {
  const int64_t i = (int64_t)blockIdx.x * blockDim.x + threadIdx.x;
  if (i < n) p[i] = v;
}
__global__ void k_fill_int2(int2 *p, int64_t n, int2 v) {
  const int64_t i = (int64_t)blockIdx.x * blockDim.x + threadIdx.x;
  if (i < n) p[i] = v;
}

__global__ void k_runs(const uint32_t *__restrict__ key, const int32_t *__restrict__ headf, const int32_t *__restrict__ hs,
                       const int32_t *__restrict__ hrun0, const int32_t *__restrict__ run_base, int item_bits, int64_t N,
                       int32_t *__restrict__ run_item_c, int32_t *__restrict__ run_item, int32_t *__restrict__ runs_per_item) {
  const int64_t p = (int64_t)blockIdx.x * blockDim.x + threadIdx.x;
  if (p >= N || !headf[p]) return;
  const uint32_t k = key[p];
  const int g = (int)(k >> item_bits);
  const int32_t item = (int32_t)(k & ((1u << item_bits) - 1u));
  const int32_t kc = hs[p] - 1;
  run_item_c[kc] = item;
  run_item[run_base[g] + kc - hrun0[g]] = item;
  atomicAdd(&runs_per_item[item], 1);
}

__global__ void k_first(const int32_t *__restrict__ hs, const int32_t *__restrict__ rowcut, const int32_t *__restrict__ hrun0,
                        const int32_t *__restrict__ run_base, int G, int R, int NT, int32_t *__restrict__ first_run) {
  const int i = blockIdx.x * blockDim.x + threadIdx.x;
  if (i >= G * NT) return;
  const int g = i / NT, t = i % NT;
  const int32_t fill = rowcut[g + 1] - rowcut[g], s0 = t * R;
  const int32_t nr = hrun0[g + 1] - hrun0[g];
  first_run[i] = run_base[g] + (s0 >= fill ? nr : hs[rowcut[g] + s0] - 1 - hrun0[g]);
}

__global__ void k_pack(const uint16_t *__restrict__ uid, const int32_t *__restrict__ headf, const int32_t *__restrict__ rowcut, int G, int R,
                       int NT, int umax, uint32_t *__restrict__ uidw, uint32_t *__restrict__ headw) {
  const int HW = R / 16, UW = 5 * HW;
  const int64_t i = (int64_t)blockIdx.x * blockDim.x + threadIdx.x;
  if (i >= (int64_t)G * HW * NT) return;
  const int t = (int)(i % NT), grp = (int)((i / NT) % HW), g = (int)(i / ((int64_t)NT * HW));
  const int64_t cap = (int64_t)R * NT;
  const int32_t fill = rowcut[g + 1] - rowcut[g];
  uint32_t w[5] = {0, 0, 0, 0, 0}, hw = 0;
  for (int q = 0; q < 16; q++) {
    const int32_t sidx = t * R + 16 * grp + q;
    const uint16_t u16 = uid[(int64_t)g * cap + sidx];
    const uint32_t u = u16 == 0xffffu ? (uint32_t)(umax - 1) : u16;
    const int bb = q / 4, k = q % 4;
    if (k < 3) {
      w[bb] |= u << (10 * k);
    } else {
      w[bb] |= (u & 3u) << 30;
      w[4] |= (u >> 2) << (8 * bb);
    }
    const bool head = sidx < fill ? headf[rowcut[g] + sidx] != 0 : sidx == fill;
    if (head || sidx == 0) hw |= 1u << q;
  }
  for (int k = 0; k < 5; k++) uidw[((int64_t)g * UW + 5 * grp + k) * NT + t] = w[k];
  headw[((int64_t)g * HW + grp) * NT + t] = hw;
}

__global__ void k_user_desc(const int32_t *__restrict__ users, const int32_t *__restrict__ empties, const int32_t *__restrict__ ucut,
                            const int32_t *__restrict__ uptr, const int32_t *__restrict__ group, int G, int32_t n_users, int32_t n_emp,
                            int2 *__restrict__ desc) {
  __shared__ int32_t cut[1026];
  for (int i = threadIdx.x; i <= G; i += blockDim.x) cut[i] = ucut[i];
  __syncthreads();
  const int32_t i = blockIdx.x * blockDim.x + threadIdx.x;
  if (i < n_users) {
    const int g = upper_group(cut, G, i);
    const int32_t j = users[i];
    desc[uptr[g] + (i - cut[g])] = make_int2(j, group ? group[j] : 0);
  } else if (i < n_users + n_emp) {
    const int32_t k = i - n_users;
    const int g = k % G;
    const int32_t j = empties[k];
    desc[uptr[g] + (cut[g + 1] - cut[g]) + k / G] = make_int2(j, group ? group[j] : 0);
  }
}

__global__ void k_item_desc(const int32_t *__restrict__ scols, const int32_t *__restrict__ group, int32_t n_items, int2 *__restrict__ desc) {
  const int32_t i = blockIdx.x * blockDim.x + threadIdx.x;
  if (i < n_items) desc[i] = make_int2(scols[i], group ? group[scols[i]] : 0);
}

__global__ void k_run_feat(const int32_t *__restrict__ run_item, const int32_t *__restrict__ scols, int32_t n_items, int64_t n_run_item,
                           int64_t n, int32_t *__restrict__ run_feat) {
  const int64_t r = (int64_t)blockIdx.x * blockDim.x + threadIdx.x;
  if (r >= n) return;
  int32_t f = -1;
  if (r < n_run_item) {
    const int32_t c = run_item[r];
    if (c < n_items) f = scols[c];
  }
  run_feat[r] = f;
}

__global__ void k_slice_keys(const int32_t *__restrict__ run_item_c, const int32_t *__restrict__ iptr, int G, int64_t n, uint32_t *__restrict__ key,
                             int32_t *__restrict__ val) {
  __shared__ int32_t cut[1026];
  for (int i = threadIdx.x; i <= G; i += blockDim.x) cut[i] = iptr[i];
  __syncthreads();
  const int64_t k = (int64_t)blockIdx.x * blockDim.x + threadIdx.x;
  if (k >= n) return;
  key[k] = (uint32_t)upper_group(cut, G, run_item_c[k]);
  val[k] = (int32_t)k;
}

__global__ void k_entries(const uint32_t *__restrict__ key, const int32_t *__restrict__ val, const int32_t *__restrict__ run_item_c,
                          const int32_t *__restrict__ hrun0, const int32_t *__restrict__ run_base, const int32_t *__restrict__ iptr,
                          const int32_t *__restrict__ eptr, const int32_t *__restrict__ sstart, int G, int64_t n, int2 *__restrict__ entries) {
  __shared__ int32_t cut[1026];
  for (int i = threadIdx.x; i <= G; i += blockDim.x) cut[i] = hrun0[i];
  __syncthreads();
  const int64_t q = (int64_t)blockIdx.x * blockDim.x + threadIdx.x;
  if (q >= n) return;
  const int sl = (int)key[q];
  const int32_t kc = val[q];
  const int g = upper_group(cut, G, kc);
  entries[eptr[sl] + (q - sstart[sl])] = make_int2(run_base[g] + (kc - cut[g]), run_item_c[kc] - iptr[sl]);
}

template <class T>
static inline std::vector<T> download(const T *p, size_t n, hipStream_t s) {
  std::vector<T> h(n);
  if (n) MFM_HIP_CHECK(hipMemcpyAsync(h.data(), p, n * sizeof(T), hipMemcpyDeviceToHost, s));
  MFM_HIP_CHECK(hipStreamSynchronize(s));
  return h;
}

static inline void inclusive_sum(const int32_t *in, int32_t *out, int64_t n, DevBuf<char> &tmp, hipStream_t s) {
  size_t bytes = 0;
  MFM_HIP_CHECK(hipcub::DeviceScan::InclusiveSum(nullptr, bytes, in, out, (int)n, s));
  if (tmp.n < bytes) tmp.alloc(bytes);
  MFM_HIP_CHECK(hipcub::DeviceScan::InclusiveSum(tmp.p, bytes, in, out, (int)n, s));
}
static inline void exclusive_sum(const int32_t *in, int32_t *out, int64_t n, DevBuf<char> &tmp, hipStream_t s) {
  size_t bytes = 0;
  MFM_HIP_CHECK(hipcub::DeviceScan::ExclusiveSum(nullptr, bytes, in, out, (int)n, s));
  if (tmp.n < bytes) tmp.alloc(bytes);
  MFM_HIP_CHECK(hipcub::DeviceScan::ExclusiveSum(tmp.p, bytes, in, out, (int)n, s));
}
static inline void sort_pairs(DevBuf<uint32_t> &k_in, DevBuf<uint32_t> &k_out, DevBuf<int32_t> &v_in, DevBuf<int32_t> &v_out, int64_t n, int bits,
                              DevBuf<char> &tmp, hipStream_t s) {
  size_t bytes = 0;
  MFM_HIP_CHECK(hipcub::DeviceRadixSort::SortPairs(nullptr, bytes, k_in.p, k_out.p, v_in.p, v_out.p, (int)n, 0, bits, s));
  if (tmp.n < bytes) tmp.alloc(bytes);
  MFM_HIP_CHECK(hipcub::DeviceRadixSort::SortPairs(tmp.p, bytes, k_in.p, k_out.p, v_in.p, v_out.p, (int)n, 0, bits, s));
}

}

static inline bool res_plan_build_device(ResPlan &rpn, const DevSparse &X, const std::vector<int32_t> *group_of, int n_cu, hipStream_t s,
                                         const std::vector<int32_t> *glevel = nullptr, const std::vector<char> *draw_empty = nullptr) {
  using namespace rp;
  rpn.ready = false;
  const int64_t N = X.rows, D0 = X.cols;
  const int NT = rpn.NT;
  rpn.n_rows = N;
  if (N < 1 || n_cu < 1 || D0 < 2 || !X.unit || X.ell_width != 2) return rpn.fail("shape");
  if (N >= ((int64_t)1 << 31) - 1) return rpn.fail("too many rows");
  auto grid = [](int64_t n) { return dim3((unsigned)((n + TB - 1) / TB)); };
  const bool tlog = env_flag("MFM_SETUP_TIMING");
  double t_prev = std::chrono::duration<double>(std::chrono::steady_clock::now().time_since_epoch()).count();
  auto lap = [&](const char *what) {
    if (!tlog) return;
    MFM_HIP_CHECK(hipStreamSynchronize(s));
    const double t = std::chrono::duration<double>(std::chrono::steady_clock::now().time_since_epoch()).count();
    std::fprintf(stderr, "[res_plan_build_device] %-34s %7.2f ms\n", what, (t - t_prev) * 1e3);
    t_prev = t;
  };
  DevBuf<char> tmp;
  DevBuf<int32_t> bflag, ucnt, icnt, red, iflag, eflag, iord, eord, uord1;
  bflag.alloc((size_t)N);
  uord1.alloc((size_t)N);
  ucnt.alloc_zero((size_t)D0, s);
  icnt.alloc_zero((size_t)D0, s);
  iflag.alloc((size_t)D0 + 1);
  eflag.alloc((size_t)D0 + 1);
  iord.alloc((size_t)D0 + 1);
  eord.alloc((size_t)D0 + 1);
  {
    const int32_t r0[4] = {-1, 0x7fffffff, 0, 0};
    red.upload(r0, 4);
  }
  lap("allocations");
  if (tlog) {
    hipLaunchKernelGGL(k_fill32, dim3(1), dim3(TB), 0, s, red.p + 3, (int64_t)1, 0);
    lap("first kernel of the library (code object load)");
  }
  hipLaunchKernelGGL(k_rows, grid(N), dim3(TB), 0, s, X.colidx.p, N, bflag.p, ucnt.p, icnt.p, red.p);
  lap("k_rows");
  const bool given = glevel && draw_empty && (int64_t)glevel->size() == D0 && (int64_t)draw_empty->size() == D0;
  if ((glevel || draw_empty) && !given) return rpn.fail("shape");
  if (given) {
    DevBuf<int32_t> d_level, d_de;
    d_level.upload(*glevel);
    std::vector<int32_t> de32(draw_empty->begin(), draw_empty->end());
    d_de.upload(de32);
    hipLaunchKernelGGL(k_cols_given, grid(D0), dim3(TB), 0, s, ucnt.p, icnt.p, d_level.p, d_de.p, D0, iflag.p, eflag.p, red.p);
    MFM_HIP_CHECK(hipStreamSynchronize(s));
  } else {
    hipLaunchKernelGGL(k_cols, grid(D0), dim3(TB), 0, s, ucnt.p, icnt.p, D0, iflag.p, eflag.p, red.p);
  }
  MFM_HIP_CHECK(hipMemsetAsync(iflag.p + D0, 0, sizeof(int32_t), s));
  MFM_HIP_CHECK(hipMemsetAsync(eflag.p + D0, 0, sizeof(int32_t), s));
  exclusive_sum(iflag.p, iord.p, D0 + 1, tmp, s);
  exclusive_sum(eflag.p, eord.p, D0 + 1, tmp, s);
  inclusive_sum(bflag.p, uord1.p, N, tmp, s);
  lap("rows, columns, scans (enqueued + run)");
  int32_t h_red[4], n_items = 0, n_emp = 0, n_users = 0;
  MFM_HIP_CHECK(hipMemcpyAsync(h_red, red.p, sizeof h_red, hipMemcpyDeviceToHost, s));
  MFM_HIP_CHECK(hipMemcpyAsync(&n_items, iord.p + D0, sizeof(int32_t), hipMemcpyDeviceToHost, s));
  MFM_HIP_CHECK(hipMemcpyAsync(&n_emp, eord.p + D0, sizeof(int32_t), hipMemcpyDeviceToHost, s));
  MFM_HIP_CHECK(hipMemcpyAsync(&n_users, uord1.p + (N - 1), sizeof(int32_t), hipMemcpyDeviceToHost, s));
  MFM_HIP_CHECK(hipStreamSynchronize(s));
  if (!given && h_red[0] >= h_red[1]) return rpn.fail("the two fields' column ranges overlap");
  if (h_red[2] != 0) return rpn.fail("first level not contiguous");
  if (n_users < 1 || n_items < 1) return rpn.fail("empty level");
  rpn.n_items = n_items;
  DevBuf<int32_t> empties, d_ustart, d_users;
  rpn.scols.alloc((size_t)n_items);
  empties.alloc((size_t)std::max(n_emp, 1));
  d_ustart.alloc((size_t)n_users + 1);
  d_users.alloc((size_t)n_users);
  hipLaunchKernelGGL(k_col_lists, grid(D0), dim3(TB), 0, s, iflag.p, eflag.p, iord.p, eord.p, D0, rpn.scols.p, empties.p);
  hipLaunchKernelGGL(k_users, grid(N), dim3(TB), 0, s, X.colidx.p, bflag.p, uord1.p, N, d_ustart.p, d_users.p);
  std::vector<int64_t> ustart((size_t)n_users + 1), ucut;
  int64_t max_user = 0;
  {
    const std::vector<int32_t> u32 = download(d_ustart.p, (size_t)n_users + 1, s);
    for (size_t u = 0; u < u32.size(); u++) ustart[u] = u32[u];
    for (int32_t u = 0; u < n_users; u++) max_user = std::max(max_user, ustart[u + 1] - ustart[u]);
  }
  if (!rpn.choose_layout(N, ustart, max_user, n_cu, ucut)) return false;
  const int G = rpn.G, R = rpn.R();
  const int64_t cap_slots = (int64_t)NT * R;
  if (G > 1024) return rpn.fail("more than 1024 workgroups");
  std::vector<int32_t> h_rowcut((size_t)G + 1), h_ucut((size_t)G + 1), h_uptr((size_t)G + 1, 0);
  int maxu = 0;
  for (int g = 0; g <= G; g++) {
    h_rowcut[g] = (int32_t)ustart[ucut[g]];
    h_ucut[g] = (int32_t)ucut[g];
  }
  for (int g = 0; g < G; g++) {
    const int nu = (int)(ucut[g + 1] - ucut[g]) + n_emp / G + (g < n_emp % G ? 1 : 0);
    maxu = std::max(maxu, nu);
    h_uptr[g + 1] = h_uptr[g] + nu;
  }
  if (maxu > NT) return rpn.fail("more first-level columns in a workgroup than threads");
  rpn.item_bits = ResPlan::bits_for((int64_t)n_items + 1);
  const int gbits = ResPlan::bits_for(G);
  if (rpn.item_bits + gbits > 32) return rpn.fail("sort key width");
  DevBuf<int32_t> rowcut, d_ucut, hrun0, hs, headf;
  rowcut.upload(h_rowcut);
  d_ucut.upload(h_ucut);
  rpn.wg_user_ptr.upload(h_uptr);
  DevBuf<uint32_t> key, key2;
  DevBuf<int32_t> val, val2;
  key.alloc((size_t)N);
  key2.alloc((size_t)N);
  val.alloc((size_t)N);
  val2.alloc((size_t)N);
  hipLaunchKernelGGL(k_keys, grid(N), dim3(TB), 0, s, X.colidx.p, iord.p, rowcut.p, G, rpn.item_bits, N, key.p, val.p);
  sort_pairs(key, key2, val, val2, N, rpn.item_bits + gbits, tmp, s);
  lap("users, cuts, keys, sort");
  DevBuf<uint16_t> uid;
  uid.alloc((size_t)G * cap_slots);
  MFM_HIP_CHECK(hipMemsetAsync(uid.p, 0xff, (size_t)G * cap_slots * sizeof(uint16_t), s));
  rpn.perm.alloc((size_t)G * cap_slots);
  MFM_HIP_CHECK(hipMemsetAsync(rpn.perm.p, 0xff, (size_t)G * cap_slots * sizeof(int32_t), s));
  headf.alloc((size_t)N);
  hs.alloc((size_t)N);
  hipLaunchKernelGGL(k_slots, grid(N), dim3(TB), 0, s, key2.p, val2.p, uord1.p, rowcut.p, d_ucut.p, rpn.item_bits, R, NT, N, rpn.perm.p, uid.p,
                     headf.p);
  inclusive_sum(headf.p, hs.p, N, tmp, s);
  hrun0.alloc((size_t)G + 1);
  hipLaunchKernelGGL(k_wg_runs, dim3((G + 1 + TB - 1) / TB), dim3(TB), 0, s, hs.p, rowcut.p, G, hrun0.p);
  const std::vector<int32_t> h_hrun0 = download(hrun0.p, (size_t)G + 1, s);
  std::vector<int32_t> nruns((size_t)G);
  for (int g = 0; g < G; g++) nruns[g] = h_hrun0[g + 1] - h_hrun0[g];
  const int64_t counter = h_hrun0[G];
  rpn.n_runs = counter;
  if (counter >= ((int64_t)1 << 31) - 2) return rpn.fail("too many runs");
  const std::vector<int32_t> run_base = ResPlan::run_bases(nruns);
  const int32_t zero_run = run_base[G];
  rpn.wg_run_ptr.upload(run_base);
  rpn.wg_nruns.upload(nruns);
  rpn.run_item.alloc((size_t)zero_run + 1);
  hipLaunchKernelGGL(k_fill32, grid(zero_run + 1), dim3(TB), 0, s, rpn.run_item.p, (int64_t)zero_run + 1, n_items);
  DevBuf<int32_t> run_item_c, runs_per_item;
  run_item_c.alloc((size_t)std::max<int64_t>(counter, 1));
  runs_per_item.alloc_zero((size_t)n_items, s);
  hipLaunchKernelGGL(k_runs, grid(N), dim3(TB), 0, s, key2.p, headf.p, hs.p, hrun0.p, rpn.wg_run_ptr.p, rpn.item_bits, N, run_item_c.p,
                     rpn.run_item.p, runs_per_item.p);
  rpn.first_run.alloc((size_t)G * NT);
  hipLaunchKernelGGL(k_first, grid((int64_t)G * NT), dim3(TB), 0, s, hs.p, rowcut.p, hrun0.p, rpn.wg_run_ptr.p, G, R, NT, rpn.first_run.p);
  lap("slots, heads, runs, first");
  std::vector<int32_t> h_slot_ptr((size_t)n_items + 1, 0), h_iptr;
  {
    const std::vector<int32_t> rpi = download(runs_per_item.p, (size_t)n_items, s);
    for (int c = 0; c < n_items; c++) h_slot_ptr[(size_t)c + 1] = h_slot_ptr[c] + rpi[c];
  }
  if (!rpn.choose_item_slices(h_slot_ptr, counter, h_iptr)) return false;
  int imax = 0;
  for (int g = 0; g < G; g++) imax = std::max(imax, h_iptr[g + 1] - h_iptr[g]);
  rpn.umax = std::max(maxu, imax) + 1;
  if (rpn.umax > 1024) return rpn.fail("internal: user field");
  const int UW = 5 * (R / 16), HW = R / 16;
  rpn.uidw.alloc((size_t)G * UW * NT);
  rpn.headw.alloc((size_t)G * HW * NT);
  hipLaunchKernelGGL(k_pack, grid((int64_t)G * HW * NT), dim3(TB), 0, s, uid.p, headf.p, rowcut.p, G, R, NT, rpn.umax, rpn.uidw.p, rpn.headw.p);
  std::vector<int32_t> h_eptr((size_t)G + 1, 0), h_sstart((size_t)G + 1, 0);
  for (int g = 0; g < G; g++) {
    const int64_t cnt = h_slot_ptr[h_iptr[g + 1]] - h_slot_ptr[h_iptr[g]];
    const int64_t e = h_eptr[g] + ((cnt + WAVE - 1) / WAVE) * WAVE;
    if (e >= ((int64_t)1 << 31)) return rpn.fail("too many entries");
    h_eptr[g + 1] = (int32_t)e;
    h_sstart[g + 1] = h_sstart[g] + (int32_t)cnt;
  }
  rpn.wg_item_ptr.upload(h_iptr);
  rpn.ent_ptr.upload(h_eptr);
  rpn.entries.alloc((size_t)h_eptr[G]);
  if (h_eptr[G]) hipLaunchKernelGGL(k_fill_int2, grid(h_eptr[G]), dim3(TB), 0, s, rpn.entries.p, (int64_t)h_eptr[G], make_int2(zero_run, 0));
  if (counter > 0) {
    DevBuf<int32_t> sstart;
    sstart.upload(h_sstart);
    DevBuf<uint32_t> sk, sk2;
    DevBuf<int32_t> sv, sv2;
    sk.alloc((size_t)counter);
    sk2.alloc((size_t)counter);
    sv.alloc((size_t)counter);
    sv2.alloc((size_t)counter);
    hipLaunchKernelGGL(k_slice_keys, grid(counter), dim3(TB), 0, s, run_item_c.p, rpn.wg_item_ptr.p, G, counter, sk.p, sv.p);
    sort_pairs(sk, sk2, sv, sv2, counter, gbits, tmp, s);
    hipLaunchKernelGGL(k_entries, grid(counter), dim3(TB), 0, s, sk2.p, sv2.p, run_item_c.p, hrun0.p, rpn.wg_run_ptr.p, rpn.wg_item_ptr.p,
                       rpn.ent_ptr.p, sstart.p, G, counter, rpn.entries.p);
    MFM_HIP_CHECK(hipStreamSynchronize(s));
  }
  lap("slices, pack, entries");
  DevBuf<int32_t> d_group;
  if (group_of && (int64_t)group_of->size() >= D0) d_group.upload(group_of->data(), (size_t)D0);
  rpn.user_desc.alloc((size_t)h_uptr[G]);
  hipLaunchKernelGGL(k_user_desc, grid((int64_t)n_users + n_emp), dim3(TB), 0, s, d_users.p, empties.p, d_ucut.p, rpn.wg_user_ptr.p, d_group.p, G,
                     n_users, n_emp, rpn.user_desc.p);
  rpn.item_desc.alloc((size_t)n_items);
  hipLaunchKernelGGL(k_item_desc, grid(n_items), dim3(TB), 0, s, rpn.scols.p, d_group.p, n_items, rpn.item_desc.p);
  rpn.run_feat.alloc((size_t)zero_run + 1 + 8);
  hipLaunchKernelGGL(k_run_feat, grid((int64_t)zero_run + 9), dim3(TB), 0, s, rpn.run_item.p, rpn.scols.p, n_items, (int64_t)zero_run + 1,
                     (int64_t)zero_run + 9, rpn.run_feat.p);
  {
    std::vector<int32_t> h_fill((size_t)G);
    for (int g = 0; g < G; g++) h_fill[g] = h_rowcut[g + 1] - h_rowcut[g];
    rpn.wg_fill.upload(h_fill);
  }
  rpn.lds_bytes = (size_t)rpn.RL * NT * 8 + (size_t)2 * (NT / WAVE) * rpn.umax * 8 + (size_t)rpn.umax * 16 + (size_t)(NT / WAVE) * 16 +
                  (NT / WAVE) * 4 + 64;
  if (rpn.lds_bytes > 160 * 1024 - 512) return rpn.fail("LDS");
  rpn.e_slots.alloc((size_t)G * cap_slots);
  rpn.sums.alloc((size_t)G);
  rpn.y_slots = DevBuf<double>();
  rpn.h_nruns = nruns;
  rpn.h_diag.clear();
  rpn.partials.alloc((size_t)2 * ((size_t)zero_run + 1));
  MFM_HIP_CHECK(hipMemsetAsync(rpn.partials.p, 0, (size_t)16 * ((size_t)zero_run + 1), s));
  rpn.dv.alloc((size_t)2 * (n_items + 1));
  rpn.bar.alloc(RES_BAR_WORDS);
  MFM_HIP_CHECK(hipStreamSynchronize(s));
  MFM_HIP_CHECK(hipGetLastError());
  lap("descriptors, buffers");
  rpn.ready = true;
  rpn.why.clear();
  return true;
}

static inline std::string res_plan_compare(const ResPlan &a, const ResPlan &b, hipStream_t s) {
  if (a.G != b.G || a.RV != b.RV || a.RL != b.RL || a.RX != b.RX || a.umax != b.umax || a.item_bits != b.item_bits || a.n_items != b.n_items ||
      a.n_rows != b.n_rows || a.n_runs != b.n_runs || a.lds_bytes != b.lds_bytes)
    return "scalars";
  auto same = [&](const void *p, size_t np, const void *q, size_t nq, size_t elem) {
    if (np != nq) return false;
    std::vector<char> x(np * elem), y(nq * elem);
    if (np) {
      MFM_HIP_CHECK(hipMemcpyAsync(x.data(), p, np * elem, hipMemcpyDeviceToHost, s));
      MFM_HIP_CHECK(hipMemcpyAsync(y.data(), q, nq * elem, hipMemcpyDeviceToHost, s));
    }
    MFM_HIP_CHECK(hipStreamSynchronize(s));
    return x == y;
  };
#define MFM_RP_CMP(f) \
  if (!same(a.f.p, a.f.n, b.f.p, b.f.n, sizeof(*a.f.p))) return #f;
  MFM_RP_CMP(perm)
  MFM_RP_CMP(first_run)
  MFM_RP_CMP(wg_run_ptr)
  MFM_RP_CMP(wg_nruns)
  MFM_RP_CMP(wg_user_ptr)
  MFM_RP_CMP(wg_item_ptr)
  MFM_RP_CMP(ent_ptr)
  MFM_RP_CMP(scols)
  MFM_RP_CMP(entries)
  MFM_RP_CMP(uidw)
  MFM_RP_CMP(headw)
  MFM_RP_CMP(run_item)
  MFM_RP_CMP(user_desc)
  MFM_RP_CMP(item_desc)
  MFM_RP_CMP(run_feat)
  MFM_RP_CMP(wg_fill)
#undef MFM_RP_CMP
  return "";
}

}
```

Baseline: 339.5.

## Replace grid-wide item reduction with class-partitioned two-level reduction and class barriers

Workgroups are split into up to eight classes. Each class reduces its own runs' partials into per-item class sums, using run-range tables that are read directly instead of a precomputed entry list, and synchronises only through a per-class barrier. A grid barrier then lets item owners add up the class sums. The aim is to replace the global scatter-gather entry list and its grid-wide barrier with cheaper class-local synchronisation and better locality. It adds an extra barrier, a cls_sum buffer, more LDS, and drops the release fence from the grid barrier. The chunk size is also raised from 4 to 8.

```diff
diff --git a/myfm_amd/csrc/mfm_res.hpp b/myfm_amd/csrc/mfm_res.hpp
--- a/myfm_amd/csrc/mfm_res.hpp
+++ b/myfm_amd/csrc/mfm_res.hpp
@@ -13,9 +13,10 @@
 namespace mfm {
 
 #ifndef MFM_RES_CH
-#define MFM_RES_CH 4
+#define MFM_RES_CH 8
 #endif
 constexpr int RES_MAX_PEERS = 8;
+constexpr int RES_PROF_W = 72;
 
 struct ResArgs {
   double2 *eq;
@@ -31,8 +32,12 @@
   const int32_t *wg_user_ptr;
   const int2 *user_desc;
   const int32_t *wg_item_ptr;
-  const int32_t *ent_ptr;
-  const int2 *entries;
+  int n_cls, cls_mm;
+  const int32_t *cls_task_ptr;
+  const int2 *cls_items;
+  const int2 *cls_tab;
+  double *cls_sum;
+  int cls_wb;
   const int32_t *scols;
   const int2 *item_desc;
   double *partials;
@@ -74,10 +79,14 @@
   __hip_atomic_store(p + 1, b, __ATOMIC_RELAXED, __HIP_MEMORY_SCOPE_AGENT);
 }
 
-enum { RES_BAR_START = 0, RES_BAR_TOP = 16, RES_BAR_XCNT = 32, RES_BAR_GEN = 160, RES_BAR_CENSUS = 288, RES_BAR_WORDS = 416 };
+enum {
+  RES_BAR_START = 0, RES_BAR_TOP = 16, RES_BAR_XCNT = 32, RES_BAR_GEN = 160, RES_BAR_CENSUS = 288, RES_BAR_CLS = 416,
+  RES_BAR_CMASK = 544, RES_BAR_WORDS = 672
+};
 struct ResBar {
   int xcc;
   unsigned long long n_x, nx;
+  bool cls_wb;
 };
 
 __device__ __forceinline__ bool res_spin(const ResArgs &a, const unsigned long long *w, unsigned long long target, bool &dead) {
@@ -113,15 +122,17 @@
   return true;
 }
 
-__device__ __forceinline__ void res_bar_init(const ResArgs &a, ResBar &rb, bool &dead) {
+__device__ __forceinline__ void res_bar_init(const ResArgs &a, int cls, ResBar &rb, bool &dead) {
   unsigned x;
   asm volatile("s_getreg_b32 %0, hwreg(HW_REG_XCC_ID, 0, 4)" : "=s"(x));
   rb.xcc = (int)(x & 7u);
   __hip_atomic_fetch_add(a.bar + RES_BAR_CENSUS + 16 * rb.xcc, 1ull, __ATOMIC_RELAXED, __HIP_MEMORY_SCOPE_AGENT);
+  __hip_atomic_fetch_or(a.bar + RES_BAR_CMASK + 16 * cls, 1ull << rb.xcc, __ATOMIC_RELAXED, __HIP_MEMORY_SCOPE_AGENT);
   asm volatile("s_waitcnt vmcnt(0)" ::: "memory");
   __hip_atomic_fetch_add(a.bar + RES_BAR_START, 1ull, __ATOMIC_RELAXED, __HIP_MEMORY_SCOPE_AGENT);
   rb.n_x = 1;
   rb.nx = 1;
+  rb.cls_wb = true;
   if (!res_spin(a, a.bar + RES_BAR_START, (unsigned long long)a.n_wg, dead)) return;
   rb.nx = 0;
   for (int i = 0; i < 8; i++) {
@@ -129,6 +140,12 @@
     rb.nx += c > 0 ? 1 : 0;
     if (i == rb.xcc) rb.n_x = c;
   }
+  bool split = a.cls_wb != 0;
+  for (int c = 0; c < a.n_cls; c++) {
+    const unsigned long long m = __hip_atomic_load(a.bar + RES_BAR_CMASK + 16 * c, __ATOMIC_RELAXED, __HIP_MEMORY_SCOPE_AGENT);
+    split = split || __builtin_popcountll(m) > 1;
+  }
+  rb.cls_wb = split;
 }
 
 __device__ __forceinline__ void res_grid_barrier(const ResArgs &a, const ResBar &rb, unsigned long long k, int tid, bool &dead) {
@@ -138,8 +155,6 @@
     const unsigned long long old =
         __hip_atomic_fetch_add(a.bar + RES_BAR_XCNT + 16 * rb.xcc, 1ull, __ATOMIC_RELAXED, __HIP_MEMORY_SCOPE_AGENT);
     if (old + 1 == k * rb.n_x) {
-      __builtin_amdgcn_fence(__ATOMIC_RELEASE, "agent");
-      asm volatile("s_waitcnt vmcnt(0)" ::: "memory");
       __hip_atomic_fetch_add(a.bar + RES_BAR_TOP, 1ull, __ATOMIC_RELAXED, __HIP_MEMORY_SCOPE_AGENT);
       if (res_spin(a, a.bar + RES_BAR_TOP, k * rb.nx, dead))
         __hip_atomic_store(a.bar + RES_BAR_GEN + 16 * rb.xcc, k, __ATOMIC_RELAXED, __HIP_MEMORY_SCOPE_AGENT);
@@ -147,6 +162,23 @@
       res_spin(a, a.bar + RES_BAR_GEN + 16 * rb.xcc, k, dead);
     }
     __builtin_amdgcn_fence(__ATOMIC_ACQUIRE, "agent");
+  }
+  __syncthreads();
+}
+
+__device__ __forceinline__ void res_class_barrier(const ResArgs &a, const ResBar &rb, int cls, unsigned long long k,
+                                                  unsigned long long n_c, int tid, bool &dead) {
+  asm volatile("s_waitcnt vmcnt(0)" ::: "memory");
+  __syncthreads();
+  if (tid == 0 && !dead) {
+    if (rb.cls_wb) {
+      __builtin_amdgcn_fence(__ATOMIC_RELEASE, "agent");
+      asm volatile("s_waitcnt vmcnt(0)" ::: "memory");
+    }
+    __hip_atomic_fetch_add(a.bar + RES_BAR_CLS + 16 * cls, 1ull, __ATOMIC_RELAXED, __HIP_MEMORY_SCOPE_AGENT);
+    res_spin(a, a.bar + RES_BAR_CLS + 16 * cls, k * n_c, dead);
+    __builtin_amdgcn_fence(__ATOMIC_ACQUIRE, "agent");
+    asm volatile("s_waitcnt vmcnt(0)" ::: "memory");
   }
   __syncthreads();
 }
@@ -170,6 +202,7 @@
   d2_t *utab = (d2_t *)(acc2 + NW * U);
   d2_t *wcarry = utab + U;
   int *wflag = (int *)(wcarry + NW);
+  int2 *ctab = (int2 *)(wflag + NW);
   const int32_t *perm_g = a.perm + (int64_t)g * Rt * NT;
   const d2_t *dv2 = (const d2_t *)a.dv;
   const int u0 = a.wg_user_ptr[g], nu = a.wg_user_ptr[g + 1] - u0;
@@ -180,10 +213,15 @@
   ResBar rbar;
   rbar.xcc = 0;
   rbar.n_x = rbar.nx = 1;
+  rbar.cls_wb = true;
+  const int cls = g % a.n_cls, MM = a.cls_mm;
+  const unsigned long long n_cls_wg = (unsigned long long)((a.n_wg - cls + a.n_cls - 1) / a.n_cls);
+  const int tk0 = a.cls_task_ptr[g], tk1 = a.cls_task_ptr[g + 1];
+  const int zero_run = a.wg_run_ptr[a.n_wg];
 #define RES_STAMP0(k) \
-  if (a.prof && tid == 0) a.prof[(int64_t)g * a.n_sw * 64 + 56 + (k)] = __builtin_amdgcn_s_memrealtime()
+  if (a.prof && tid == 0) a.prof[(int64_t)g * a.n_sw * RES_PROF_W + 56 + (k)] = __builtin_amdgcn_s_memrealtime()
   RES_STAMP0(0);
-  if (tid == 0) res_bar_init(a, rbar, dead);
+  if (tid == 0) res_bar_init(a, cls, rbar, dead);
   RES_STAMP0(1);
   const int wv_hi = wv >> 2;
 #define RES_PRIO(j)                  \
@@ -193,10 +231,11 @@
     __builtin_amdgcn_s_setprio(0)
   const int trash_run = a.wg_run_ptr[g] + a.wg_nruns[g];
 #define RES_STAMP(k)                                                                                      \
-  if (a.prof && tid == 0) a.prof[((int64_t)g * a.n_sw + (f - f_first)) * 64 + (k)] = __builtin_amdgcn_s_memrealtime()
+  if (a.prof && tid == 0) a.prof[((int64_t)g * a.n_sw + (f - f_first)) * RES_PROF_W + (k)] = __builtin_amdgcn_s_memrealtime()
 
   for (int i = tid; i < 2 * NW * U; i += NT) acc1[i] = 0.0;
   for (int i = tid; i < U; i += NT) utab[i] = d2_t{0.0, 0.0};
+  if (tk0 < tk1 && tid <= MM) ctab[tid] = a.cls_tab[(int64_t)tk0 * (MM + 1) + tid];
 
   res_u4_t uw[NG];
   unsigned ux[NG];
@@ -527,11 +566,11 @@
           for (int bp = 0; bp < 2; bp++) {
               RES_STEP_B(j, 2 * bp, itA, itB, ccA, ccB);
             if (a.prof && lane == 0 && (wv == 4 || wv == 7))
-              a.prof[((int64_t)g * a.n_sw + (f - f_first)) * 64 + 16 + (wv == 4 ? 0 : 20) + 4 * j + 2 * bp] =
+              a.prof[((int64_t)g * a.n_sw + (f - f_first)) * RES_PROF_W + 16 + (wv == 4 ? 0 : 20) + 4 * j + 2 * bp] =
                   __builtin_amdgcn_s_memrealtime();
             RES_STEP_B(j, 2 * bp + 1, itB, itA, ccB, ccA);
             if (a.prof && lane == 0 && (wv == 4 || wv == 7))
-              a.prof[((int64_t)g * a.n_sw + (f - f_first)) * 64 + 16 + (wv == 4 ? 0 : 20) + 4 * j + 2 * bp + 1] =
+              a.prof[((int64_t)g * a.n_sw + (f - f_first)) * RES_PROF_W + 16 + (wv == 4 ? 0 : 20) + 4 * j + 2 * bp + 1] =
                   __builtin_amdgcn_s_memrealtime();
           }
         }
@@ -562,7 +601,7 @@
 #undef RES_PARTIAL_STORE
       }
       if (a.prof && lane == 0)
-        a.prof[((int64_t)g * a.n_sw + (f - f_first)) * 64 + 8 + wv] = __builtin_amdgcn_s_memrealtime();
+        a.prof[((int64_t)g * a.n_sw + (f - f_first)) * RES_PROF_W + 64 + wv] = __builtin_amdgcn_s_memrealtime();
       double v1 = s1, v2 = s2;
       int fl = have_head ? 1 : 0;
       wave_segscan2(v1, v2, fl);
@@ -595,10 +634,7 @@
       }
     }
     RES_STAMP(3);
-    constexpr int CH = MFM_RES_CH;
-    const int c0 = a.ent_ptr[g] >> 6, c1 = a.ent_ptr[g + 1] >> 6;
-    const int per = (c1 - c0 + NW - 1) / NW;
-    const int wb = c0 + wv * per, we = wb + per < c1 ? wb + per : c1;
+    constexpr int CHC = MFM_RES_CH;
     const int i0 = a.wg_item_ptr[g], ni = a.wg_item_ptr[g + 1] - i0;
     const bool more = f + 1 < a.f_end;
     int ij = 0;
@@ -612,44 +648,76 @@
       ilam = lamf[d.y];
       imu = muf[d.y];
     }
-    int2 en[CH];
-#pragma unroll
-    for (int k = 0; k < CH; k++) en[k] = make_int2(0, 0);
-    if (wb < we) {
-#pragma unroll
-      for (int k = 0; k < CH; k++) en[k] = a.entries[(int64_t)(wb + k < we ? wb + k : wb) * WAVE + lane];
-    }
-    res_grid_barrier(a, rbar, ++nbar, tid, dead);
+    res_class_barrier(a, rbar, cls, (unsigned long long)(f - f_first) + 1ull, n_cls_wg, tid, dead);
     RES_STAMP(4);
     {
       const d2_t *part2 = (const d2_t *)a.partials;
-      for (int cb = wb; cb < we; cb += CH) {
-        d2_t sv[CH];
-#pragma unroll
-        for (int k = 0; k < CH; k++) sv[k] = part2[en[k].x];
-        int il[CH];
-#pragma unroll
-        for (int k = 0; k < CH; k++) il[k] = en[k].y;
-        if (cb + CH < we) {
-#pragma unroll
-          for (int k = 0; k < CH; k++) en[k] = a.entries[(int64_t)(cb + CH + k < we ? cb + CH + k : cb + CH) * WAVE + lane];
-        }
-#pragma unroll
-        for (int k = 0; k < CH; k++) {
-          if (cb + k >= we) break;
-          __hip_atomic_fetch_add(&acc1[wv * U + il[k]], sv[k][0], __ATOMIC_RELAXED, __HIP_MEMORY_SCOPE_WORKGROUP);
-          __hip_atomic_fetch_add(&acc2[wv * U + il[k]], sv[k][1], __ATOMIC_RELAXED, __HIP_MEMORY_SCOPE_WORKGROUP);
-        }
-      }
-      __syncthreads();
+      for (int tk = tk0; tk < tk1; tk++) {
+        const int2 ci = a.cls_items[tk];
+        const int T = ctab[MM].y;
+        const int nch = (T + WAVE - 1) / WAVE, per = (nch + NW - 1) / NW;
+        const int wb = wv * per, we = wb + per < nch ? wb + per : nch;
+        int src = 0;
+        for (int cb = wb; cb < we; cb += CHC) {
+          d2_t sv[CHC];
+          int it[CHC];
+#pragma unroll
+          for (int k = 0; k < CHC; k++) {
+            const int p = (cb + k) * WAVE + lane;
+            int run = zero_run;
+            if (cb + k < we && p < T) {
+              while (ctab[src + 1].y <= p) src++;
+              run = ctab[src].x + (p - ctab[src].y);
+            }
+            sv[k] = part2[run];
+            it[k] = a.run_item[run];
+          }
+#pragma unroll
+          for (int k = 0; k < CHC; k++) {
+            if (cb + k < we && (cb + k) * WAVE + lane < T) {
+              __hip_atomic_fetch_add(&acc1[wv * U + (it[k] - ci.x)], sv[k][0], __ATOMIC_RELAXED, __HIP_MEMORY_SCOPE_WORKGROUP);
+              __hip_atomic_fetch_add(&acc2[wv * U + (it[k] - ci.x)], sv[k][1], __ATOMIC_RELAXED, __HIP_MEMORY_SCOPE_WORKGROUP);
+            }
+          }
+        }
+        __syncthreads();
+        if (tid < ci.y - ci.x) {
+          double S1 = 0.0, S2 = 0.0;
+#pragma unroll
+          for (int w = 0; w < NW; w++) {
+            S1 += acc1[w * U + tid];
+            S2 += acc2[w * U + tid];
+            acc1[w * U + tid] = 0.0;
+            acc2[w * U + tid] = 0.0;
+          }
+          res_store2(a.cls_sum + 2 * ((int64_t)cls * a.n_items + ci.x + tid), S1, S2);
+        }
+        if (tk1 - tk0 > 1 && tid <= MM) {
+          const int tn = tk + 1 < tk1 ? tk + 1 : tk0;
+          ctab[tid] = a.cls_tab[(int64_t)tn * (MM + 1) + tid];
+        }
+        __syncthreads();
+      }
+    }
+    RES_STAMP(5);
+    res_grid_barrier(a, rbar, ++nbar, tid, dead);
+    RES_STAMP(6);
+    {
       double S1 = 0.0, S2 = 0.0;
       if (tid < ni) {
-#pragma unroll
-        for (int w = 0; w < NW; w++) {
-          S1 += acc1[w * U + tid];
-          S2 += acc2[w * U + tid];
-          acc1[w * U + tid] = 0.0;
-          acc2[w * U + tid] = 0.0;
+        double c1[8], c2[8];
+#pragma unroll
+        for (int c = 0; c < 8; c++) {
+          const double *q = a.cls_sum + 2 * ((int64_t)(c < a.n_cls ? c : 0) * a.n_items + i0 + tid);
+          c1[c] = __hip_atomic_load(q, __ATOMIC_RELAXED, __HIP_MEMORY_SCOPE_AGENT);
+          c2[c] = __hip_atomic_load(q + 1, __ATOMIC_RELAXED, __HIP_MEMORY_SCOPE_AGENT);
+        }
+#pragma unroll
+        for (int c = 0; c < 8; c++) {
+          if (c < a.n_cls) {
+            S1 += c1[c];
+            S2 += c2[c];
+          }
         }
       }
       if (XCH) {
@@ -688,9 +756,9 @@
         res_store2(a.dv + 2 * (int64_t)(i0 + tid), fresh - iold, ivn);
       }
     }
-    RES_STAMP(5);
+    RES_STAMP(7);
     res_grid_barrier(a, rbar, ++nbar, tid, dead);
-    RES_STAMP(6);
+    RES_STAMP(8);
   }
 #undef RES_STAMP
   RES_STAMP0(3);
@@ -974,8 +1042,11 @@
   bool allow_overflow = true;
   int64_t n_rows = 0, n_runs = 0;
   size_t lds_bytes = 0;
-  DevBuf<int32_t> perm, first_run, wg_run_ptr, wg_nruns, wg_user_ptr, wg_item_ptr, ent_ptr, scols;
-  DevBuf<int2> entries;
+  DevBuf<int32_t> perm, first_run, wg_run_ptr, wg_nruns, wg_user_ptr, wg_item_ptr, scols;
+  int n_cls = 0, cls_mm = 0;
+  DevBuf<int32_t> cls_task_ptr;
+  DevBuf<int2> cls_items, cls_tab;
+  DevBuf<double> cls_sum;
   DevBuf<uint32_t> uidw, headw;
   DevBuf<int32_t> run_item;
   DevBuf<int2> user_desc, item_desc;
@@ -1112,27 +1183,60 @@
     if (!found) return fail("no variant fits (rows per CU, or a first-level column longer than a workgroup's capacity)");
     return true;
   }
-  bool choose_item_slices(const std::vector<int32_t> &slot_ptr, int64_t counter, std::vector<int32_t> &iptr) {
-    iptr.assign((size_t)G + 1, 0);
+  static bool slice_items(const std::vector<int32_t> &prefix, int n_items, int parts, int cap, double per_item, std::vector<int32_t> &ptr) {
+    ptr.assign((size_t)parts + 1, 0);
     bool ok = false;
     for (double scale = 1.0; scale < 3.0 && !ok; scale *= 1.1) {
-      const double target = scale * ((double)counter + 16.0 * n_items) / G;
+      const double target = scale * ((double)prefix[n_items] + per_item * n_items) / parts;
       double acc = 0.0;
       int gq = 0, cnt = 0;
       for (int c = 0; c < n_items; c++) {
-        acc += (double)(slot_ptr[c + 1] - slot_ptr[c]) + 16.0;
+        acc += (double)(prefix[c + 1] - prefix[c]) + per_item;
         cnt++;
-        if ((acc >= target || cnt == NT) && gq + 1 < G) {
-          iptr[++gq] = c + 1;
+        if ((acc >= target || cnt == cap) && gq + 1 < parts) {
+          ptr[++gq] = c + 1;
           acc = 0.0;
           cnt = 0;
         }
       }
-      ok = cnt <= NT;
-      for (gq++; gq <= G; gq++) iptr[gq] = n_items;
-    }
-    if (!ok) return fail("more second-level columns than the workgroups can draw");
+      ok = cnt <= cap;
+      for (gq++; gq <= parts; gq++) ptr[gq] = n_items;
+    }
+    return ok;
+  }
+  bool choose_item_slices(const std::vector<int32_t> &slot_ptr, std::vector<int32_t> &iptr) {
+    if (!slice_items(slot_ptr, n_items, G, NT, 16.0, iptr)) return fail("more second-level columns than the workgroups can draw");
     return true;
+  }
+  bool choose_classes(const std::vector<int32_t> &cnt, std::vector<int32_t> &tptr, std::vector<int2> &titems) {
+    n_cls = std::min(G, 8);
+    cls_mm = (G + n_cls - 1) / n_cls;
+    if (cls_mm > 64) return fail("internal: class size");
+    std::vector<std::vector<int2>> tasks((size_t)G);
+    std::vector<int32_t> prefix((size_t)n_items + 1), ptr;
+    for (int c = 0; c < n_cls; c++) {
+      const int m = (G - c + n_cls - 1) / n_cls;
+      prefix[0] = 0;
+      for (int i = 0; i < n_items; i++) prefix[(size_t)i + 1] = prefix[i] + cnt[(size_t)c * n_items + i];
+      int k = 1;
+      while (!slice_items(prefix, n_items, k * m, umax - 1, 4.0, ptr)) {
+        if (k * m > n_items) return fail("internal: class reduction tasks");
+        k++;
+      }
+      for (int q = 0; q < m; q++)
+        for (int t = q * k; t < (q + 1) * k; t++) tasks[(size_t)c + (size_t)q * n_cls].push_back(make_int2(ptr[t], ptr[t + 1]));
+    }
+    tptr.assign((size_t)G + 1, 0);
+    titems.clear();
+    for (int g = 0; g < G; g++) {
+      titems.insert(titems.end(), tasks[g].begin(), tasks[g].end());
+      tptr[(size_t)g + 1] = (int32_t)titems.size();
+    }
+    return true;
+  }
+  size_t lds_need() const {
+    return (size_t)RL * NT * 8 + (size_t)2 * (NT / WAVE) * umax * 8 + (size_t)umax * 16 + (size_t)(NT / WAVE) * 16 + (NT / WAVE) * 4 +
+           (size_t)8 * (cls_mm + 1) + 64;
   }
   static std::vector<int32_t> run_bases(const std::vector<int32_t> &nruns) {
     const int G = (int)nruns.size();
@@ -1281,7 +1385,7 @@
       h_uptr[g + 1] = (int32_t)h_udesc.size();
     }
     std::vector<int32_t> h_iptr;
-    if (!choose_item_slices(h_slot_ptr, counter, h_iptr)) return false;
+    if (!choose_item_slices(h_slot_ptr, h_iptr)) return false;
     int imax = 0;
     for (int g = 0; g < G; g++) imax = std::max(imax, h_iptr[g + 1] - h_iptr[g]);
     umax = std::max(maxu, imax) + 1;
@@ -1302,33 +1406,33 @@
       }
     });
     h_uid = std::vector<uint16_t>();
-    std::vector<int32_t> slice_of((size_t)n_items);
-    for (int g = 0; g < G; g++)
-      for (int c = h_iptr[g]; c < h_iptr[g + 1]; c++) slice_of[c] = g;
-    std::vector<int32_t> h_eptr((size_t)G + 1, 0);
+    std::vector<int32_t> h_tptr;
+    std::vector<int2> h_titems, h_ctab;
     {
-      std::vector<int64_t> cnt((size_t)G, 0);
+      std::vector<int32_t> ccnt((size_t)std::min(G, 8) * n_items, 0);
       for (int g = 0; g < G; g++)
-        for (int32_t c : wg_run_item[g]) cnt[slice_of[c]]++;
-      for (int g = 0; g < G; g++) {
-        const int64_t e = h_eptr[g] + ((cnt[g] + WAVE - 1) / WAVE) * WAVE;
-        if (e >= ((int64_t)1 << 31)) return fail("too many entries");
-        h_eptr[g + 1] = (int32_t)e;
-      }
-    }
-    std::vector<int2> h_entries((size_t)h_eptr[G], make_int2(zero_run, 0));
-    {
-      std::vector<int64_t> pos((size_t)G);
-      for (int g = 0; g < G; g++) pos[g] = h_eptr[g];
+        for (int32_t c : wg_run_item[g]) ccnt[(size_t)(g % std::min(G, 8)) * n_items + c]++;
+      if (!choose_classes(ccnt, h_tptr, h_titems)) return false;
+      h_ctab.assign(h_titems.size() * (size_t)(cls_mm + 1), make_int2(0, 0));
       for (int g = 0; g < G; g++)
-        for (size_t l = 0; l < wg_run_item[g].size(); l++) {
-          const int32_t c = wg_run_item[g][l];
-          const int sgl = slice_of[c];
-          h_entries[(size_t)pos[sgl]++] = make_int2(run_base[g] + (int32_t)l, c - h_iptr[sgl]);
-        }
-    }
-    if (h_entries.size() >= ((size_t)1 << 31)) return fail("too many entries");
-    lds_bytes = (size_t)RL * NT * 8 + (size_t)2 * (NT / WAVE) * umax * 8 + (size_t)umax * 16 + (size_t)(NT / WAVE) * 16 + (NT / WAVE) * 4 + 64;
+        for (int t = h_tptr[g]; t < h_tptr[g + 1]; t++) {
+          int32_t pos = 0;
+          for (int k = 0; k < cls_mm; k++) {
+            const int sg = g % n_cls + k * n_cls;
+            int2 e = make_int2(0, pos);
+            if (sg < G) {
+              const std::vector<int32_t> &ri = wg_run_item[sg];
+              const int32_t lo = (int32_t)(std::lower_bound(ri.begin(), ri.end(), h_titems[t].x) - ri.begin());
+              const int32_t hi = (int32_t)(std::lower_bound(ri.begin(), ri.end(), h_titems[t].y) - ri.begin());
+              e.x = run_base[sg] + lo;
+              pos += hi - lo;
+            }
+            h_ctab[(size_t)t * (cls_mm + 1) + k] = e;
+          }
+          h_ctab[(size_t)t * (cls_mm + 1) + cls_mm] = make_int2(0, pos);
+        }
+    }
+    lds_bytes = lds_need();
     if (lds_bytes > 160 * 1024 - 512) return fail("LDS");
     uidw.upload(h_uidw);
     headw.upload(h_headw);
@@ -1338,8 +1442,9 @@
     wg_user_ptr.upload(h_uptr);
     user_desc.upload(h_udesc.data(), h_udesc.size());
     wg_item_ptr.upload(h_iptr);
-    ent_ptr.upload(h_eptr);
-    entries.upload(h_entries.data(), h_entries.size());
+    cls_task_ptr.upload(h_tptr);
+    cls_items.upload(h_titems.data(), h_titems.size());
+    cls_tab.upload(h_ctab.data(), h_ctab.size());
     wg_run_ptr.upload(run_base);
     wg_nruns.upload(nruns);
     e_slots.alloc((size_t)G * cap_slots);
@@ -1400,6 +1505,7 @@
     partials.alloc((size_t)2 * ((size_t)zero_run + 1));
     MFM_HIP_CHECK(hipMemset(partials.p, 0, (size_t)16 * ((size_t)zero_run + 1)));
     dv.alloc((size_t)2 * (n_items + 1));
+    cls_sum.alloc((size_t)2 * n_cls * n_items);
     bar.alloc(RES_BAR_WORDS);
     ready = true;
     why.clear();
@@ -1457,8 +1563,13 @@
   a.wg_user_ptr = rp.wg_user_ptr.p;
   a.user_desc = rp.user_desc.p;
   a.wg_item_ptr = rp.wg_item_ptr.p;
-  a.ent_ptr = rp.ent_ptr.p;
-  a.entries = rp.entries.p;
+  a.n_cls = rp.n_cls;
+  a.cls_mm = rp.cls_mm;
+  a.cls_task_ptr = rp.cls_task_ptr.p;
+  a.cls_items = rp.cls_items.p;
+  a.cls_tab = rp.cls_tab.p;
+  a.cls_sum = rp.cls_sum.p;
+  a.cls_wb = env_flag("MFM_RES_CLASS_WB") ? 1 : 0;
   a.wg_run_ptr = rp.wg_run_ptr.p;
   a.wg_nruns = rp.wg_nruns.p;
   a.scols = rp.scols.p;
@@ -1498,12 +1609,13 @@
   const bool prof = env_flag("MFM_RES_PROF") && ++prof_launch == env_int("MFM_RES_PROF", 0);
   DevBuf<unsigned long long> prof_buf;
   if (prof) {
-    prof_buf.alloc((size_t)rp.G * a.n_sw * 64);
-    MFM_HIP_CHECK(hipMemsetAsync(prof_buf.p, 0, (size_t)rp.G * a.n_sw * 512, s));
+    prof_buf.alloc((size_t)rp.G * a.n_sw * RES_PROF_W);
+    MFM_HIP_CHECK(hipMemsetAsync(prof_buf.p, 0, (size_t)rp.G * a.n_sw * RES_PROF_W * 8, s));
     a.prof = prof_buf.p;
   }
   const int K = a.n_sw;
-  double bytes = (8.0 + (load_slots ? 0.0 : 4.0) + 1.4 + (no_store ? 0.0 : 8.0)) * rp.n_rows + K * 48.0 * rp.n_runs;
+  double bytes = (8.0 + (load_slots ? 0.0 : 4.0) + 1.4 + (no_store ? 0.0 : 8.0)) * rp.n_rows +
+                 K * (44.0 * rp.n_runs + 32.0 * rp.n_cls * rp.n_items);
   if (rp.RX) bytes += (double)K * (16.0 + 1.75) * (double)rp.G * rp.NT * rp.RX;
   hipLaunchKernelGGL(k_res_init_dv, dim3((rp.n_items + 256) / 256), dim3(256), 0, s,
                      w ? (const double *)nullptr : V + (int64_t)f_begin * D, rp.scols.p, rp.n_items,
@@ -1551,16 +1663,18 @@
   if (prof) {
     MFM_HIP_CHECK(hipStreamSynchronize(s));
     const int K2 = a.n_sw;
-    std::vector<unsigned long long> h((size_t)rp.G * K2 * 64);
+    std::vector<unsigned long long> h((size_t)rp.G * K2 * RES_PROF_W);
     MFM_HIP_CHECK(hipMemcpy(h.data(), prof_buf.p, h.size() * 8, hipMemcpyDeviceToHost));
-    const char *names[6] = {"sweep A", "user draw", "sweep B", "barrier 1 (wait)", "item draw", "barrier 2 (wait)"};
+    constexpr int NPH = 8;
+    const char *names[NPH] = {"sweep A", "user draw", "sweep B", "class barrier", "class reduction", "barrier 1 (wait)", "item draw",
+                              "barrier 2 (wait)"};
     std::fprintf(stderr, "[resident profile] G=%d factors=%d; us per factor: mean | mean of max over workgroups | mean of min\n", rp.G, K2);
-    for (int ph = 0; ph < 6; ph++) {
+    for (int ph = 0; ph < NPH; ph++) {
       double sm = 0, smax = 0, smin = 0;
       for (int f = 0; f < K2; f++) {
         double mx = 0, mn = 1e30;
         for (int g = 0; g < rp.G; g++) {
-          const unsigned long long *t = &h[((size_t)g * K2 + f) * 64];
+          const unsigned long long *t = &h[((size_t)g * K2 + f) * RES_PROF_W];
           const double d = (double)(t[ph + 1] - t[ph]) * 0.01;
           sm += d;
           mx = std::max(mx, d);
@@ -1575,7 +1689,7 @@
       std::vector<std::pair<double, int>> tb;
       for (int g = 0; g < rp.G; g++) {
         double d = 0;
-        for (int f = 0; f < K2; f++) d += (double)(h[((size_t)g * K2 + f) * 64 + 3] - h[((size_t)g * K2 + f) * 64 + 2]) * 0.01;
+        for (int f = 0; f < K2; f++) d += (double)(h[((size_t)g * K2 + f) * RES_PROF_W + 3] - h[((size_t)g * K2 + f) * RES_PROF_W + 2]) * 0.01;
         tb.push_back({d / K2, g});
       }
       std::sort(tb.begin(), tb.end());
@@ -1591,14 +1705,14 @@
           std::fprintf(stderr, "    wg %d %.1f us: %s; waves:", g, tb[k].first, rp.h_diag[g].c_str());
           for (int w = 0; w < 8; w++) {
             double d = 0;
-            for (int f = 0; f < K2; f++) d += (double)(h[((size_t)g * K2 + f) * 64 + 8 + w] - h[((size_t)g * K2 + f) * 64 + 2]) * 0.01;
+            for (int f = 0; f < K2; f++) d += (double)(h[((size_t)g * K2 + f) * RES_PROF_W + 64 + w] - h[((size_t)g * K2 + f) * RES_PROF_W + 2]) * 0.01;
             std::fprintf(stderr, " %.1f", d / K2);
           }
           std::fprintf(stderr, "\n      batches of waves 4 and 7 (factor 3 alone):");
           for (int w : {0, 20}) {
             std::fprintf(stderr, " |");
             for (int b = 0; b < (rp.RV + rp.RL) / 4; b++)
-              std::fprintf(stderr, " %.1f", (double)(h[((size_t)g * K2 + 3) * 64 + 16 + w + b] - h[((size_t)g * K2 + 3) * 64 + 2]) * 0.01);
+              std::fprintf(stderr, " %.1f", (double)(h[((size_t)g * K2 + 3) * RES_PROF_W + 16 + w + b] - h[((size_t)g * K2 + 3) * RES_PROF_W + 2]) * 0.01);
           }
           std::fprintf(stderr, "\n");
         }
@@ -1607,9 +1721,9 @@
       if (FILE *fp = std::fopen(dump, "w")) {
         for (int g = 0; g < rp.G; g++) {
           std::fprintf(fp, "%d", g);
-          for (int ph = 0; ph < 6; ph++) {
+          for (int ph = 0; ph < NPH; ph++) {
             double d = 0;
-            for (int f = 0; f < K2; f++) d += (double)(h[((size_t)g * K2 + f) * 64 + ph + 1] - h[((size_t)g * K2 + f) * 64 + ph]) * 0.01;
+            for (int f = 0; f < K2; f++) d += (double)(h[((size_t)g * K2 + f) * RES_PROF_W + ph + 1] - h[((size_t)g * K2 + f) * RES_PROF_W + ph]) * 0.01;
             std::fprintf(fp, " %.2f", d / K2);
           }
           std::fprintf(fp, " | %s\n", rp.h_diag.empty() ? "" : rp.h_diag[g].c_str());
@@ -1622,7 +1736,7 @@
       for (int ph = 0; ph < 4; ph++) {
         double sm = 0, mx = 0;
         for (int g = 0; g < rp.G; g++) {
-          const double d = (double)(h[(size_t)g * K2 * 64 + 56 + ph + 1] - h[(size_t)g * K2 * 64 + 56 + ph]) * 0.01;
+          const double d = (double)(h[(size_t)g * K2 * RES_PROF_W + 56 + ph + 1] - h[(size_t)g * K2 * RES_PROF_W + 56 + ph]) * 0.01;
           sm += d;
           mx = std::max(mx, d);
         }
@@ -1630,13 +1744,13 @@
       }
       unsigned long long t0 = ~0ull, t1 = 0;
       for (int g = 0; g < rp.G; g++) {
-        t0 = std::min(t0, h[(size_t)g * K2 * 64 + 56]);
-        t1 = std::max(t1, h[(size_t)g * K2 * 64 + 60]);
+        t0 = std::min(t0, h[(size_t)g * K2 * RES_PROF_W + 56]);
+        t1 = std::max(t1, h[(size_t)g * K2 * RES_PROF_W + 60]);
       }
       std::fprintf(stderr, "  first workgroup in to last workgroup out: %.1f us\n", (double)(t1 - t0) * 0.01);
     }
     double tot = 0;
-    for (int g = 0; g < rp.G; g++) tot += (double)(h[((size_t)g * K2 + K2 - 1) * 64 + 6] - h[(size_t)g * K2 * 64]) * 0.01;
+    for (int g = 0; g < rp.G; g++) tot += (double)(h[((size_t)g * K2 + K2 - 1) * RES_PROF_W + NPH] - h[(size_t)g * K2 * RES_PROF_W]) * 0.01;
     std::fprintf(stderr, "  factors, start to end: %.1f us (%.2f per factor)\n", tot / rp.G, tot / rp.G / K2);
   }
 }
diff --git a/myfm_amd/csrc/mfm_res_plan.hpp b/myfm_amd/csrc/mfm_res_plan.hpp
--- a/myfm_amd/csrc/mfm_res_plan.hpp
+++ b/myfm_amd/csrc/mfm_res_plan.hpp
@@ -121,10 +121,6 @@
 }
 
 __global__ void k_fill32(int32_t *p, int64_t n, int32_t v) {
-  const int64_t i = (int64_t)blockIdx.x * blockDim.x + threadIdx.x;
-  if (i < n) p[i] = v;
-}
-__global__ void k_fill_int2(int2 *p, int64_t n, int2 v) {
   const int64_t i = (int64_t)blockIdx.x * blockDim.x + threadIdx.x;
   if (i < n) p[i] = v;
 }
@@ -216,29 +212,46 @@
   run_feat[r] = f;
 }
 
-__global__ void k_slice_keys(const int32_t *__restrict__ run_item_c, const int32_t *__restrict__ iptr, int G, int64_t n, uint32_t *__restrict__ key,
-                             int32_t *__restrict__ val) {
+__global__ void k_cls_count(const int32_t *__restrict__ run_item_c, const int32_t *__restrict__ hrun0, int G, int n_cls, int n_items, int64_t n,
+                            int32_t *__restrict__ cnt) {
   __shared__ int32_t cut[1026];
-  for (int i = threadIdx.x; i <= G; i += blockDim.x) cut[i] = iptr[i];
+  for (int i = threadIdx.x; i <= G; i += blockDim.x) cut[i] = hrun0[i];
   __syncthreads();
   const int64_t k = (int64_t)blockIdx.x * blockDim.x + threadIdx.x;
   if (k >= n) return;
-  key[k] = (uint32_t)upper_group(cut, G, run_item_c[k]);
-  val[k] = (int32_t)k;
-}
-
-__global__ void k_entries(const uint32_t *__restrict__ key, const int32_t *__restrict__ val, const int32_t *__restrict__ run_item_c,
-                          const int32_t *__restrict__ hrun0, const int32_t *__restrict__ run_base, const int32_t *__restrict__ iptr,
-                          const int32_t *__restrict__ eptr, const int32_t *__restrict__ sstart, int G, int64_t n, int2 *__restrict__ entries) {
-  __shared__ int32_t cut[1026];
-  for (int i = threadIdx.x; i <= G; i += blockDim.x) cut[i] = hrun0[i];
-  __syncthreads();
-  const int64_t q = (int64_t)blockIdx.x * blockDim.x + threadIdx.x;
-  if (q >= n) return;
-  const int sl = (int)key[q];
-  const int32_t kc = val[q];
-  const int g = upper_group(cut, G, kc);
-  entries[eptr[sl] + (q - sstart[sl])] = make_int2(run_base[g] + (kc - cut[g]), run_item_c[kc] - iptr[sl]);
+  const int g = upper_group(cut, G, (int32_t)k);
+  atomicAdd(&cnt[(int64_t)(g % n_cls) * n_items + run_item_c[k]], 1);
+}
+
+__global__ void k_cls_tab(const int2 *__restrict__ titems, const int32_t *__restrict__ tcls, const int32_t *__restrict__ run_item,
+                          const int32_t *__restrict__ run_base, const int32_t *__restrict__ nruns, int G, int n_cls, int mm, int n_tasks,
+                          int2 *__restrict__ tab) {
+  const int t = blockIdx.x * blockDim.x + threadIdx.x;
+  if (t >= n_tasks) return;
+  const int2 ti = titems[t];
+  auto lower = [&](int32_t b, int32_t e, int32_t item) {
+    while (b < e) {
+      const int32_t mid = b + ((e - b) >> 1);
+      if (run_item[mid] < item)
+        b = mid + 1;
+      else
+        e = mid;
+    }
+    return b;
+  };
+  int32_t pos = 0;
+  for (int k = 0; k < mm; k++) {
+    const int sg = tcls[t] + k * n_cls;
+    int2 e = make_int2(0, pos);
+    if (sg < G) {
+      const int32_t b = run_base[sg], end = b + nruns[sg];
+      const int32_t lo = lower(b, end, ti.x), hi = lower(lo, end, ti.y);
+      e.x = lo;
+      pos += hi - lo;
+    }
+    tab[(int64_t)t * (mm + 1) + k] = e;
+  }
+  tab[(int64_t)t * (mm + 1) + mm] = make_int2(0, pos);
 }
 
 template <class T>
@@ -422,7 +435,7 @@
     const std::vector<int32_t> rpi = download(runs_per_item.p, (size_t)n_items, s);
     for (int c = 0; c < n_items; c++) h_slot_ptr[(size_t)c + 1] = h_slot_ptr[c] + rpi[c];
   }
-  if (!rpn.choose_item_slices(h_slot_ptr, counter, h_iptr)) return false;
+  if (!rpn.choose_item_slices(h_slot_ptr, h_iptr)) return false;
   int imax = 0;
   for (int g = 0; g < G; g++) imax = std::max(imax, h_iptr[g + 1] - h_iptr[g]);
   rpn.umax = std::max(maxu, imax) + 1;
@@ -431,34 +444,30 @@
   rpn.uidw.alloc((size_t)G * UW * NT);
   rpn.headw.alloc((size_t)G * HW * NT);
   hipLaunchKernelGGL(k_pack, grid((int64_t)G * HW * NT), dim3(TB), 0, s, uid.p, headf.p, rowcut.p, G, R, NT, rpn.umax, rpn.uidw.p, rpn.headw.p);
-  std::vector<int32_t> h_eptr((size_t)G + 1, 0), h_sstart((size_t)G + 1, 0);
-  for (int g = 0; g < G; g++) {
-    const int64_t cnt = h_slot_ptr[h_iptr[g + 1]] - h_slot_ptr[h_iptr[g]];
-    const int64_t e = h_eptr[g] + ((cnt + WAVE - 1) / WAVE) * WAVE;
-    if (e >= ((int64_t)1 << 31)) return rpn.fail("too many entries");
-    h_eptr[g + 1] = (int32_t)e;
-    h_sstart[g + 1] = h_sstart[g] + (int32_t)cnt;
-  }
   rpn.wg_item_ptr.upload(h_iptr);
-  rpn.ent_ptr.upload(h_eptr);
-  rpn.entries.alloc((size_t)h_eptr[G]);
-  if (h_eptr[G]) hipLaunchKernelGGL(k_fill_int2, grid(h_eptr[G]), dim3(TB), 0, s, rpn.entries.p, (int64_t)h_eptr[G], make_int2(zero_run, 0));
-  if (counter > 0) {
-    DevBuf<int32_t> sstart;
-    sstart.upload(h_sstart);
-    DevBuf<uint32_t> sk, sk2;
-    DevBuf<int32_t> sv, sv2;
-    sk.alloc((size_t)counter);
-    sk2.alloc((size_t)counter);
-    sv.alloc((size_t)counter);
-    sv2.alloc((size_t)counter);
-    hipLaunchKernelGGL(k_slice_keys, grid(counter), dim3(TB), 0, s, run_item_c.p, rpn.wg_item_ptr.p, G, counter, sk.p, sv.p);
-    sort_pairs(sk, sk2, sv, sv2, counter, gbits, tmp, s);
-    hipLaunchKernelGGL(k_entries, grid(counter), dim3(TB), 0, s, sk2.p, sv2.p, run_item_c.p, hrun0.p, rpn.wg_run_ptr.p, rpn.wg_item_ptr.p,
-                       rpn.ent_ptr.p, sstart.p, G, counter, rpn.entries.p);
+  {
+    const int n_cls = std::min(G, 8);
+    DevBuf<int32_t> ccnt;
+    ccnt.alloc_zero((size_t)n_cls * n_items, s);
+    if (counter > 0)
+      hipLaunchKernelGGL(k_cls_count, grid(counter), dim3(TB), 0, s, run_item_c.p, hrun0.p, G, n_cls, n_items, counter, ccnt.p);
+    std::vector<int32_t> h_tptr;
+    std::vector<int2> h_titems;
+    if (!rpn.choose_classes(download(ccnt.p, (size_t)n_cls * n_items, s), h_tptr, h_titems)) return false;
+    std::vector<int32_t> h_tcls(h_titems.size());
+    for (int g = 0; g < G; g++)
+      for (int t = h_tptr[g]; t < h_tptr[g + 1]; t++) h_tcls[t] = g % n_cls;
+    DevBuf<int32_t> tcls;
+    tcls.upload(h_tcls);
+    rpn.cls_task_ptr.upload(h_tptr);
+    rpn.cls_items.upload(h_titems.data(), h_titems.size());
+    const int n_tasks = (int)h_titems.size();
+    rpn.cls_tab.alloc((size_t)n_tasks * (rpn.cls_mm + 1));
+    hipLaunchKernelGGL(k_cls_tab, dim3((n_tasks + TB - 1) / TB), dim3(TB), 0, s, rpn.cls_items.p, tcls.p, rpn.run_item.p, rpn.wg_run_ptr.p,
+                       rpn.wg_nruns.p, G, n_cls, rpn.cls_mm, n_tasks, rpn.cls_tab.p);
     MFM_HIP_CHECK(hipStreamSynchronize(s));
   }
-  lap("slices, pack, entries");
+  lap("slices, pack, classes");
   DevBuf<int32_t> d_group;
   if (group_of && (int64_t)group_of->size() >= D0) d_group.upload(group_of->data(), (size_t)D0);
   rpn.user_desc.alloc((size_t)h_uptr[G]);
@@ -474,8 +483,7 @@
     for (int g = 0; g < G; g++) h_fill[g] = h_rowcut[g + 1] - h_rowcut[g];
     rpn.wg_fill.upload(h_fill);
   }
-  rpn.lds_bytes = (size_t)rpn.RL * NT * 8 + (size_t)2 * (NT / WAVE) * rpn.umax * 8 + (size_t)rpn.umax * 16 + (size_t)(NT / WAVE) * 16 +
-                  (NT / WAVE) * 4 + 64;
+  rpn.lds_bytes = rpn.lds_need();
   if (rpn.lds_bytes > 160 * 1024 - 512) return rpn.fail("LDS");
   rpn.e_slots.alloc((size_t)G * cap_slots);
   rpn.sums.alloc((size_t)G);
@@ -485,6 +493,7 @@
   rpn.partials.alloc((size_t)2 * ((size_t)zero_run + 1));
   MFM_HIP_CHECK(hipMemsetAsync(rpn.partials.p, 0, (size_t)16 * ((size_t)zero_run + 1), s));
   rpn.dv.alloc((size_t)2 * (n_items + 1));
+  rpn.cls_sum.alloc((size_t)2 * rpn.n_cls * n_items);
   rpn.bar.alloc(RES_BAR_WORDS);
   MFM_HIP_CHECK(hipStreamSynchronize(s));
   MFM_HIP_CHECK(hipGetLastError());
@@ -496,7 +505,7 @@
 
 static inline std::string res_plan_compare(const ResPlan &a, const ResPlan &b, hipStream_t s) {
   if (a.G != b.G || a.RV != b.RV || a.RL != b.RL || a.RX != b.RX || a.umax != b.umax || a.item_bits != b.item_bits || a.n_items != b.n_items ||
-      a.n_rows != b.n_rows || a.n_runs != b.n_runs || a.lds_bytes != b.lds_bytes)
+      a.n_rows != b.n_rows || a.n_runs != b.n_runs || a.lds_bytes != b.lds_bytes || a.n_cls != b.n_cls || a.cls_mm != b.cls_mm)
     return "scalars";
   auto same = [&](const void *p, size_t np, const void *q, size_t nq, size_t elem) {
     if (np != nq) return false;
@@ -516,9 +525,10 @@
   MFM_RP_CMP(wg_nruns)
   MFM_RP_CMP(wg_user_ptr)
   MFM_RP_CMP(wg_item_ptr)
-  MFM_RP_CMP(ent_ptr)
+  MFM_RP_CMP(cls_task_ptr)
+  MFM_RP_CMP(cls_items)
+  MFM_RP_CMP(cls_tab)
   MFM_RP_CMP(scols)
-  MFM_RP_CMP(entries)
   MFM_RP_CMP(uidw)
   MFM_RP_CMP(headw)
   MFM_RP_CMP(run_item)
```

Result: slower. 335.5, median of 6 (-1.2%).
